# jonathanking/protein-transformer

Measured on AMD Instinct MI355X. Metric: train-step residues/sec (enc-only d512, drmsd loss), higher is better.
Workload: dtype f32 (GEMM and attention operands scaled by powers of two and split into 2 f16 terms [activation x weight products, weight-gradient products whose operands come with a uniform scale, attention with head size 64 / 32] or exactly into 3 bf16 terms [the other weight-gradient products; everything when to; 1 GPU; enc-only d_model=512 n_layers=6 n_head=8 d_ff=2048, -l drmsd, sgd lr 1e-4 wd 0.01 clip 1, dropout 0.1, 32 proteins x L=512 per GPU (BASELINE.json configs[3]); global_batch=32, seq_len=512, parallelism=dp1

## Files before the change

include/ptamd.h:

```cpp
#ifndef PTAMD_H
#define PTAMD_H

#include <stddef.h>
#include <stdint.h>

#ifdef __cplusplus
extern "C" {
#endif

#define PTAMD_OK 0
#define PTAMD_ERR_BAD_SHAPE (-1)
#define PTAMD_ERR_TOO_LONG (-2)
#define PTAMD_ERR_WORKSPACE (-3)
#define PTAMD_ERR_HIP (-4)
#define PTAMD_ERR_ALIGN (-5)

#define PTAMD_ST_BAD_RESIDUE 1
#define PTAMD_ST_TOO_SHORT 2
#define PTAMD_ST_BAD_THETA 4
#define PTAMD_ST_NONFINITE 8

#define PTAMD_PAD_ID 20
#define PTAMD_NUM_ANGLES 12
#define PTAMD_NUM_SLOTS 14
// ... 24 lines not shown

int ptamd_kabsch_rmsd(const float *pred_crd, const float *true_crd, const int64_t *seq, int B, int L, float *rmsd,
                      void *stream);

size_t ptamd_mse_angles_workspace_bytes(void);
int ptamd_mse_angles_fwd(const float *pred, const float *truth, int64_t T, float *out, void *workspace,
                         size_t workspace_bytes, void *stream);
int ptamd_mse_angles_bwd(const float *pred, const float *truth, int64_t T, const float *sums, float coef,
                         int accumulate, float *dpred, void *stream);

#define PTAMD_EPI_RELU 1
#define PTAMD_EPI_TANH 2
#define PTAMD_EPI_ACCUM 4
#define PTAMD_EPI_SLABS 16
#define PTAMD_EPI_GATE 8
typedef struct {
  int M, N, K;
  const float *A; int lda; int a_kmajor;
  const float *B; int ldb; int b_kmajor;
  float *C; int ldc;
  const float *bias;
  const float *residual; int ldr;
  int flags;
  float dropout_p; uint64_t seed; uint32_t stream_id;
  int split_k;
  void *workspace; size_t workspace_bytes;
  float *colsum;
  float gate_scale;
  int arith;
  int reserved_cus;
  const uint32_t *a_scale; int a_scale_stride;
  const uint32_t *b_scale; int b_scale_stride;
  const uint64_t *gate_mask;
} ptamd_gemm_args;
size_t ptamd_gate_mask_bytes(int M, int N);
size_t ptamd_gemm_workspace_bytes(int M, int N, int split_k);
int ptamd_gemm(const ptamd_gemm_args *args, void *stream);

#define PTAMD_GEMM_F32 0
#define PTAMD_GEMM_BF16X3 1
#define PTAMD_GEMM_BF16X3_FULL 2
#define PTAMD_GEMM_F16X2 3
#define PTAMD_GEMM_AUTO 4
int ptamd_gemm_products(const ptamd_gemm_args *args);
int ptamd_gemm_group(const ptamd_gemm_args *args, int n, void *stream);

size_t ptamd_hp_bytes(int rows, int K);
int ptamd_hp_padded_rows(int rows);
int ptamd_hp_split(const float *x, int ld, int rows, int K, int transposed, void *planes, float *scale, void *stream);
typedef struct {
  const float *x; int ld, rows, K;
  void *planes; float *scale;
} ptamd_hp_split_job;
int ptamd_hp_split_rows(const ptamd_hp_split_job *jobs_host, int njobs, void *stream);
int ptamd_hp_split_cols(const ptamd_hp_split_job *jobs_host, int njobs, void *stream);
typedef struct {
  int M, N, K;
  const void *A; const float *A_scale;
  const void *B; const float *B_scale;
  float *C; int ldc;
  const float *bias;
  const float *residual; int ldr;
  int flags;
  float dropout_p; uint64_t seed; uint32_t stream_id;
  int split_k;
  void *workspace; size_t workspace_bytes;
  float gate_scale;
  int reserved_cus;
  const uint64_t *gate_mask;
  uint64_t *gate_mask_out;
  void *kv_planes; float *kv_inv; int kv_col0, kv_heads;
} ptamd_gemm_hp_args;
size_t ptamd_gemm_hp_workspace_bytes(int M, int N, int split_k);
int ptamd_gemm_hp(const ptamd_gemm_hp_args *args, void *stream);

typedef struct {
  const float *w; int rows, cols, ld;
  uint32_t *row_scale; uint32_t *col_scale; float *stats;
  int rows_only;
} ptamd_wscale_job;
int ptamd_weight_scales(const ptamd_wscale_job *jobs_host, int njobs, void *stream);
typedef struct {
  const float *ln_gamma_stats; const float *ln_beta_stats;
  const float *w_stats; int w_stat_index;
  const float *bias_stats;
  float sqrt_d, post_scale;
  uint32_t *out_scale; float *out_value;
} ptamd_bound_job;
int ptamd_bound_scales(const ptamd_bound_job *jobs_host, int njobs, void *stream);
typedef struct { uint32_t *dst; int64_t n; uint32_t value; } ptamd_fill_job;
int ptamd_fill_u32(const ptamd_fill_job *jobs_host, int njobs, void *stream);

typedef struct {
  int64_t offset;
  int32_t rows, cols;
  int32_t stats_row0;
  int32_t stats_index;
  int32_t row_scale_index;
  int32_t col_scale_index;
  int32_t colmax_index;
  int32_t colsq_index;
  uint64_t row_planes;
  uint64_t col_planes;
  int32_t ld;
  int32_t rowmax_index;
} ptamd_wprep_seg;
typedef struct {
  int32_t ln_gamma_stats, ln_beta_stats, w_stats, w_stat_index, bias_stats;
  float sqrt_d, post_scale;
  int32_t out_scale, out_value;
} ptamd_wprep_bound;
typedef struct {
// ... 93 lines not shown
```

protein_transformer_amd/_lib.py:

```python
import ctypes as C
import os

import torch

_HERE = os.path.dirname(os.path.abspath(__file__))
_TAG = os.environ.get("PTAMD_LIB_TAG", "")
LIB_PATH = os.path.join(_HERE, "csrc", f"libptamd_{_TAG}.so" if _TAG else "libptamd.so")

OK = 0
ERRORS = {-1: "bad shape", -2: "sequence too long for the NeRF LDS staging", -3: "workspace missing or too small",
          -4: "HIP runtime error", -5: "pointer not 16-byte aligned"}
ST_BAD_RESIDUE, ST_TOO_SHORT, ST_BAD_THETA, ST_NONFINITE = 1, 2, 4, 8

_p, _i, _i64, _f, _sz, _u64, _u32 = C.c_void_p, C.c_int, C.c_int64, C.c_float, C.c_size_t, C.c_uint64, C.c_uint32


class GemmArgs(C.Structure):
    _fields_ = [("M", _i), ("N", _i), ("K", _i),
                ("A", _p), ("lda", _i), ("a_kmajor", _i),
                ("B", _p), ("ldb", _i), ("b_kmajor", _i),
                ("C", _p), ("ldc", _i),
                ("bias", _p),
                ("residual", _p), ("ldr", _i),
                ("flags", _i),
                ("dropout_p", _f), ("seed", _u64), ("stream_id", _u32),
                ("split_k", _i),
                ("workspace", _p), ("workspace_bytes", _sz),
                ("colsum", _p),
                ("gate_scale", _f),
                ("arith", _i),
                ("reserved_cus", _i),
                ("a_scale", _p), ("a_scale_stride", _i),
                ("b_scale", _p), ("b_scale_stride", _i),
                ("gate_mask", _p)]


class WScaleJob(C.Structure):
    _fields_ = [("w", _p), ("rows", _i), ("cols", _i), ("ld", _i), ("row_scale", _p), ("col_scale", _p), ("stats", _p),
                ("rows_only", _i)]


class BoundJob(C.Structure):
    _fields_ = [("ln_gamma_stats", _p), ("ln_beta_stats", _p), ("w_stats", _p), ("w_stat_index", _i), ("bias_stats", _p),
                ("sqrt_d", _f), ("post_scale", _f), ("out_scale", _p), ("out_value", _p)]


class LnReduceJob(C.Structure):
    _fields_ = [("partials", _p), ("D", _i), ("dgamma", _p), ("dbeta", _p)]


class FillJob(C.Structure):
    _fields_ = [("dst", _p), ("n", _i64), ("value", _u32)]


class HpSplitJob(C.Structure):
    _fields_ = [("x", _p), ("ld", _i), ("rows", _i), ("K", _i), ("planes", _p), ("scale", _p)]


class GemmHpArgs(C.Structure):
    _fields_ = [("M", _i), ("N", _i), ("K", _i),
                ("A", _p), ("A_scale", _p),
                ("B", _p), ("B_scale", _p),
                ("C", _p), ("ldc", _i),
                ("bias", _p),
                ("residual", _p), ("ldr", _i),
                ("flags", _i),
                ("dropout_p", _f), ("seed", _u64), ("stream_id", _u32),
                ("split_k", _i),
                ("workspace", _p), ("workspace_bytes", _sz),
                ("gate_scale", _f),
                ("reserved_cus", _i),
                ("gate_mask", _p), ("gate_mask_out", _p),
                ("kv_planes", _p), ("kv_inv", _p), ("kv_col0", _i), ("kv_heads", _i)]


class WprepSeg(C.Structure):
    _fields_ = [("offset", _i64), ("rows", C.c_int32), ("cols", C.c_int32), ("stats_row0", C.c_int32), ("stats_index", C.c_int32),
                ("row_scale_index", C.c_int32), ("col_scale_index", C.c_int32), ("colmax_index", C.c_int32),
                ("colsq_index", C.c_int32), ("row_planes", _u64), ("col_planes", _u64), ("ld", C.c_int32), ("rowmax_index", C.c_int32)]


class WprepBound(C.Structure):
    _fields_ = [("ln_gamma_stats", C.c_int32), ("ln_beta_stats", C.c_int32), ("w_stats", C.c_int32), ("w_stat_index", C.c_int32),
                ("bias_stats", C.c_int32), ("sqrt_d", _f), ("post_scale", _f), ("out_scale", C.c_int32), ("out_value", C.c_int32)]


class WprepPlan(C.Structure):
    _fields_ = [("segs", _p), ("nsegs", C.c_int32),
                ("blocks_a", _p), ("nblocks_a", C.c_int32), ("nblocks_a_matrices", C.c_int32),
                ("plain", _p), ("nplain", C.c_int32),
                ("blocks_b", _p), ("nblocks_b", C.c_int32),
                ("bounds", _p), ("nbounds", C.c_int32),
                ("groups", _p), ("ngroups", C.c_int32),
                ("colnorm_segs", _p),
                ("scales", _p), ("values", _p),
                ("colmax", _p), ("ncolmax", C.c_int32),
                ("colsq", _p),
                ("stats", _p), ("nstats", C.c_int32),
                ("numel", _i64), ("with_planes", C.c_int32)]


SIGNATURES = {
    "ptamd_version": (C.c_char_p, []),
    "ptamd_last_hip_error": (C.c_char_p, []),
    "ptamd_sidechain_atoms": (_i, [_i]),
    "ptamd_angles_fwd": (_i, [_p, _p, _i64, _p]),
# ... 133 lines not shown
```

protein_transformer_amd/csrc/gemm.hip:

```cpp
#include <stdlib.h>

#include "gemm_common.h"

namespace ptgemm {
namespace {

template <bool KMAJOR, int BK>
__device__ __forceinline__ void store_stage(float *__restrict__ s, int tid, const float4 (&v)[BK / 8]) {
  constexpr int LPR = BK / 4, LD_R = BK + 4;
#pragma unroll
  for (int i = 0; i < BK / 8; ++i) {
    if (!KMAJOR) {
      const int row = tid / LPR + (NT / LPR) * i, k = 4 * (tid % LPR);
      *reinterpret_cast<float4 *>(s + row * LD_R + k) = v[i];
    } else {
      const int k = (tid >> 5) + 8 * i, row = 4 * (tid & 31);
      *reinterpret_cast<float4 *>(s + k * LD_C + row) = v[i];
    }
  }
}
template <bool KMAJOR, int BK>
__device__ __forceinline__ void read_frag(const float *__restrict__ s, int r, int lh, int m, float (&f)[4]) {
  constexpr int LD_R = BK + 4;
  if (!KMAJOR) {
// ... 313 lines not shown
int round4(int n) { return (n + 3) & ~3; }
}

size_t ptamd_gemm_workspace_bytes(int M, int N, int split_k) {
  if (M <= 0 || N <= 0) return 0;
  return slab_bytes(M, N, split_k) + (size_t)(round4(M) + round4(N)) * sizeof(uint32_t);
}

namespace {
bool valid_arith(int mode) {
  return mode == PTAMD_GEMM_F32 || mode == PTAMD_GEMM_BF16X3 || mode == PTAMD_GEMM_BF16X3_FULL || mode == PTAMD_GEMM_F16X2 ||
         mode == PTAMD_GEMM_AUTO;
}
int resolve_mode(const ptamd_gemm_args *a) {
  int mode = a->arith;
  if (mode == PTAMD_GEMM_AUTO) mode = a->a_kmajor ? PTAMD_GEMM_BF16X3 : PTAMD_GEMM_F16X2;
  const size_t a_bytes = (size_t)(a->a_kmajor ? a->K : a->M) * a->lda * sizeof(float);
  const size_t b_bytes = (size_t)(a->b_kmajor ? a->K : a->N) * a->ldb * sizeof(float);
  if (mode == PTAMD_GEMM_F16X2 && a->K < 32) mode = PTAMD_GEMM_BF16X3;
  if (a->K < 16 || a_bytes >= ((size_t)1 << 32) || b_bytes >= ((size_t)1 << 32)) mode = PTAMD_GEMM_F32;
  return mode;
}
}

int ptamd_gemm_products(const ptamd_gemm_args *a) {
  if (!a || a->M <= 0 || a->N <= 0 || a->K <= 0 || !valid_arith(a->arith)) return PTAMD_ERR_BAD_SHAPE;
  const int mode = resolve_mode(a);
  return mode == PTAMD_GEMM_F32 ? 1 : mode == PTAMD_GEMM_F16X2 ? 3 : mode == PTAMD_GEMM_BF16X3_FULL ? 9 : 6;
}

namespace {
int build_params(const ptamd_gemm_args *a, GemmParams &p, int &splits, int &mode, float *&user_c) {
  if (!a || a->M <= 0 || a->N <= 0 || a->K <= 0 || !valid_arith(a->arith)) return PTAMD_ERR_BAD_SHAPE;
  if ((a->lda & 3) || (a->ldb & 3)) return PTAMD_ERR_BAD_SHAPE;
  if ((!a->a_kmajor || !a->b_kmajor) && (a->K & 3)) return PTAMD_ERR_BAD_SHAPE;
  if (a->a_kmajor && (a->M & 3)) return PTAMD_ERR_BAD_SHAPE;
  if (a->b_kmajor && (a->N & 3)) return PTAMD_ERR_BAD_SHAPE;
  if (!pt_aligned16(a->A) || !pt_aligned16(a->B)) return PTAMD_ERR_ALIGN;
  if (a->dropout_p < 0.f || a->dropout_p >= 1.f) return PTAMD_ERR_BAD_SHAPE;
  splits = a->split_k > 1 ? a->split_k : 1;
  constexpr int BK = 32;
  const int kblocks = (a->K + BK - 1) / BK;
  if (splits > kblocks) splits = kblocks;
  p.M = a->M; p.N = a->N; p.K = a->K;
  p.A = a->A; p.lda = a->lda; p.B = a->B; p.ldb = a->ldb; p.C = a->C; p.ldc = a->ldc;
  p.bias = a->bias; p.residual = a->residual; p.ldr = a->ldr; p.flags = a->flags & ~PTAMD_EPI_SLABS;
  if ((a->flags & PTAMD_EPI_SLABS) && (a->bias || a->residual || a->colsum || a->gate_mask || a->dropout_p != 0.f ||
                                      (a->flags & (PTAMD_EPI_RELU | PTAMD_EPI_TANH | PTAMD_EPI_ACCUM | PTAMD_EPI_GATE))))
    return PTAMD_ERR_BAD_SHAPE;
  p.dropout_p = a->dropout_p; p.seed = a->seed; p.stream_id = a->stream_id; p.gate_scale = a->gate_scale;
  p.reserved_cus = a->reserved_cus;
  p.k_per_split = ((kblocks + splits - 1) / splits) * BK;
  splits = (a->K + p.k_per_split - 1) / p.k_per_split;
  p.splits = splits;
  p.vec_epilogue = !(a->N & 3) && !(a->ldc & 3) && pt_aligned16(a->C) &&
                   (!a->residual || (!(a->ldr & 3) && pt_aligned16(a->residual))) &&
                   (splits == 1 || pt_aligned16(a->workspace));
  p.slab = 0;
  p.colsum = a->colsum;
  p.colsum_share = 1;
  {
    const int tiles_n = (a->N + BN - 1) / BN;
    while (p.colsum_share * 2 <= tiles_n && p.colsum_share < 16) p.colsum_share *= 2;
  }
  if (a->colsum && !a->a_kmajor) return PTAMD_ERR_BAD_SHAPE;
  if ((a->flags & PTAMD_EPI_GATE) && (a->residual == nullptr) == (a->gate_mask == nullptr)) return PTAMD_ERR_BAD_SHAPE;
  if (a->gate_mask && !(a->flags & PTAMD_EPI_GATE)) return PTAMD_ERR_BAD_SHAPE;
  p.gate_mask = a->gate_mask; p.gate_mask_out = nullptr;
  p.mask_rb = (a->M + 31) / 32; p.mask_cb = (a->N + 31) / 32;
  user_c = a->C;
  if (splits > 1) {
    if (!a->workspace || a->workspace_bytes < slab_bytes(a->M, a->N, splits)) return PTAMD_ERR_WORKSPACE;
    p.slab = (size_t)a->M * a->N;
    p.C = static_cast<float *>(a->workspace);
    if (a->colsum) p.colsum = p.C + (size_t)splits * p.slab;
  }
  mode = resolve_mode(a);
  if (a->gate_mask && (mode != PTAMD_GEMM_F16X2 || !p.vec_epilogue || splits > 1 || a->dropout_p != 0.f)) return PTAMD_ERR_BAD_SHAPE;
  p.scale_a = p.scale_b = nullptr;
  p.scale_a_stride = p.scale_b_stride = 1;
  if (mode == PTAMD_GEMM_F16X2) {
    if (a->a_scale && a->a_scale_stride != 0 && a->a_scale_stride != 1) return PTAMD_ERR_BAD_SHAPE;
    if (a->b_scale && a->b_scale_stride != 0 && a->b_scale_stride != 1) return PTAMD_ERR_BAD_SHAPE;
  }
  return PTAMD_OK;
}
}

size_t ptamd_gate_mask_bytes(int M, int N) {
  if (M <= 0 || N <= 0) return 0;
  return (size_t)((M + 31) / 32) * ((N + 31) / 32) * 16 * sizeof(uint64_t);
}

int ptamd_gemm(const ptamd_gemm_args *a, void *stream) {
  GemmParams p;
  int splits, mode;
  float *user_c;
  if (const int rc = build_params(a, p, splits, mode, user_c)) return rc;
  hipStream_t st = (hipStream_t)stream;
  if (mode == PTAMD_GEMM_F16X2) {
    uint32_t *sa = nullptr, *sb = nullptr;
    if (!a->a_scale || !a->b_scale) {
      if (!a->workspace || !pt_aligned16(a->workspace) || a->workspace_bytes < ptamd_gemm_workspace_bytes(a->M, a->N, splits))
        return PTAMD_ERR_WORKSPACE;
      uint32_t *ws = reinterpret_cast<uint32_t *>(static_cast<char *>(a->workspace) + slab_bytes(a->M, a->N, splits));
      if (!a->a_scale) sa = ws;
      if (!a->b_scale) sb = ws + round4(a->M);
      if (const int rs = launch_row_scales(p, a->a_kmajor != 0, a->b_kmajor != 0, sa, sb, st)) return rs;
    }
    p.scale_a = a->a_scale ? a->a_scale : sa;
// ... 60 lines not shown
```

protein_transformer_amd/csrc/gemm_common.h:

```cpp
#pragma once
#include "common.h"

namespace ptgemm {

typedef float f32x16 __attribute__((ext_vector_type(16)));
typedef float f32x4 __attribute__((ext_vector_type(4)));

constexpr int BM = 128, BN = 128, NT = 256;
constexpr int LD_C = 132;

struct GemmParams {
  int M, N, K;
  const float *A;
  int lda;
  const float *B;
  int ldb;
  float *C;
  int ldc;
  const float *bias;
  const float *residual;
  int ldr;
  int flags;
  float dropout_p;
  uint64_t seed;
  uint32_t stream_id;
  int k_per_split;
  int splits;
  size_t slab;
  int vec_epilogue;
  float *colsum;
  int colsum_share;
  float gate_scale;
  const uint32_t *scale_a, *scale_b;
  int scale_a_stride, scale_b_stride;
  int reserved_cus;
  const uint64_t *gate_mask;
  uint64_t *gate_mask_out;
  int mask_rb, mask_cb;
};
__device__ __forceinline__ uint32_t load_gate_masks(const GemmParams &p, int rb, int cb, int lane) {
  const int rbu = __builtin_amdgcn_readfirstlane(rb), cbu = __builtin_amdgcn_readfirstlane(cb);
  const bool in = rbu < p.mask_rb && cbu < p.mask_cb;
  const uint32_t *src = reinterpret_cast<const uint32_t *>(p.gate_mask + ((size_t)(in ? cbu : 0) * p.mask_rb + (in ? rbu : 0)) * 16);
  return src[lane & 31];
}
__device__ __forceinline__ bool gate_keep(uint32_t masks, int r) {
  const uint32_t lo = (uint32_t)__builtin_amdgcn_readlane((int)masks, 2 * r), hi = (uint32_t)__builtin_amdgcn_readlane((int)masks, 2 * r + 1);
  return __builtin_amdgcn_inverse_ballot_w64(((uint64_t)hi << 32) | lo);
}

template <bool KMAJOR, int BK>
__device__ __forceinline__ void load_stage(const float *__restrict__ src, int ld, int rows, int r0, int kend, int k0,
                                           int tid, float4 (&v)[BK / 8]) {
  constexpr int LPR = BK / 4;
#pragma unroll
  for (int i = 0; i < BK / 8; ++i) {
    if (!KMAJOR) {
      const int row = r0 + tid / LPR + (NT / LPR) * i, k = k0 + 4 * (tid % LPR);
      v[i] = (row < rows && k < kend) ? *reinterpret_cast<const float4 *>(src + (size_t)row * ld + k)
                                      : make_float4(0.f, 0.f, 0.f, 0.f);
    } else {
      const int k = k0 + (tid >> 5) + 8 * i, row = r0 + 4 * (tid & 31);
      v[i] = (k < kend && row < rows) ? *reinterpret_cast<const float4 *>(src + (size_t)k * ld + row)
                                      : make_float4(0.f, 0.f, 0.f, 0.f);
    }
  }
}
__device__ __forceinline__ float epilogue_value(float v, int row, int col, const GemmParams &p, uint32_t thr,
                                                float keep_scale) {
  if (p.bias) v += p.bias[col];
  if (p.flags & PTAMD_EPI_RELU) v = fmaxf(v, 0.f);
// ... 192 lines not shown
```

protein_transformer_amd/csrc/gemm_f16x2.hip:

```cpp
#include "gemm_split_kernel.h"

namespace ptgemm {
namespace {

struct ScaleJob {
  const float *x;
  int ld, rows, K, kmajor;
  uint32_t *scale;
  int blocks;
};
constexpr int RS_THREADS = 256, RS_ROWS = 8, RS_KCHUNK = 128;
constexpr int RS_KMAJOR_CHUNKS = 1, RS_KMAJOR_WHOLE = 2;

__device__ __forceinline__ float absmax4(float m, const float4 v) {
  return fmaxf(fmaxf(m, fmaxf(fabsf(v.x), fabsf(v.y))), fmaxf(fabsf(v.z), fabsf(v.w)));
}

__global__ __launch_bounds__(RS_THREADS) void gemm_row_scale_kernel(const ScaleJob ja, const ScaleJob jb) {
  const bool second = (int)blockIdx.x >= ja.blocks;
  const ScaleJob j = second ? jb : ja;
  const int b = (int)blockIdx.x - (second ? ja.blocks : 0);
  const int tid = threadIdx.x, lane = tid & 63, wave = tid >> 6;
  if (!j.kmajor) {
    for (int rr = 0; rr < RS_ROWS / 4; rr += 2) {
// ... 65 lines not shown
        m.x = fmaxf(m.x, o.x); m.y = fmaxf(m.y, o.y); m.z = fmaxf(m.z, o.z); m.w = fmaxf(m.w, o.w);
      }
      atomicMin(j.scale + r4 + 0, row_scale_bits(__float_as_uint(m.x)));
      atomicMin(j.scale + r4 + 1, row_scale_bits(__float_as_uint(m.y)));
      atomicMin(j.scale + r4 + 2, row_scale_bits(__float_as_uint(m.z)));
      atomicMin(j.scale + r4 + 3, row_scale_bits(__float_as_uint(m.w)));
    }
  }
}

}

int launch_row_scales(const GemmParams &p, bool a_kmajor, bool b_kmajor, uint32_t *scale_a, uint32_t *scale_b, hipStream_t st) {
  auto job = [](const float *x, int ld, int rows, int K, bool kmajor, uint32_t *scale) {
    const int mode = !kmajor ? 0 : ((size_t)rows * K <= ((size_t)1 << 21) ? RS_KMAJOR_WHOLE : RS_KMAJOR_CHUNKS);
    ScaleJob j = {x, ld, rows, K, mode, scale, 0};
    j.blocks = mode == RS_KMAJOR_CHUNKS  ? ((rows + 255) / 256) * ((K + RS_KCHUNK - 1) / RS_KCHUNK)
               : mode == RS_KMAJOR_WHOLE ? (rows + 15) / 16
                                         : (rows + RS_ROWS - 1) / RS_ROWS;
    return j;
  };
  ScaleJob ja = job(p.A, p.lda, p.M, p.K, a_kmajor, scale_a), jb = job(p.B, p.ldb, p.N, p.K, b_kmajor, scale_b);
  if (!scale_a) ja.blocks = 0;
  if (!scale_b) jb.blocks = 0;
  if (ja.blocks + jb.blocks == 0) return PTAMD_OK;
  if (ja.blocks && ja.kmajor == RS_KMAJOR_CHUNKS)
    PT_HIP_TRY(hipMemsetD32Async(reinterpret_cast<hipDeviceptr_t>(scale_a), (int)(254u << 23), (size_t)p.M, st));
  if (jb.blocks && jb.kmajor == RS_KMAJOR_CHUNKS)
    PT_HIP_TRY(hipMemsetD32Async(reinterpret_cast<hipDeviceptr_t>(scale_b), (int)(254u << 23), (size_t)p.N, st));
  hipLaunchKernelGGL(gemm_row_scale_kernel, dim3(ja.blocks + jb.blocks), dim3(RS_THREADS), 0, st, ja, jb);
  return pt_check_launch();
}

int launch_group_f16x2(const GemmGroup &g, hipStream_t st) { return launch_group<3>(g, st); }

int launch_split_f16x2(const GemmParams &p, bool a_kmajor, bool b_kmajor, int splits, hipStream_t st) {
  const bool plain = p.slab != 0 || (!p.bias && !p.residual && !p.flags && p.dropout_p == 0.f);
  if (plain) return launch_layout<3, EPI_PLAIN>(p, a_kmajor, b_kmajor, splits, st);
  if (p.dropout_p == 0.f) return launch_layout<3, EPI_NODROP>(p, a_kmajor, b_kmajor, splits, st);
  return launch_layout<3, EPI_FULL>(p, a_kmajor, b_kmajor, splits, st);
}

}
```

protein_transformer_amd/csrc/gemm_hp.hip:

```cpp
#include <stdlib.h>

#include "gemm_common.h"
#include "hp_format.h"
#include "kv_format.h"
#include "split_bf16.h"

extern "C" __device__ int pt_llvm_amdgcn_writelane(int value, int lane, int old) __asm("llvm.amdgcn.writelane");

namespace pthp {
namespace {

using ptgemm::GemmParams;
using ptgemm::f32x16;
using ptsplit::f16x8;

constexpr int HBN = 128;

struct HpParams {
  GemmParams g;
  const char *a_planes, *b_planes;
  const float *a_scale, *b_scale;
  int kb16;
  int a_rb_last, b_rb_last;
  char *kv_planes;
  float *kv_inv;
  int kv_col0, kv_heads, kv_nt;
};

typedef __attribute__((address_space(1))) const void *gptr_t;
typedef __attribute__((address_space(3))) void *lptr_t;
__device__ __forceinline__ void dma16(const char *g, char *l) {
  __builtin_amdgcn_global_load_lds((gptr_t)g, (lptr_t)l, 16, 0, 0);
}

struct Item {
  int bm0, bn0, z, kbeg, kend;
};
struct Cursor {
  int w, k0;
  Item it;
};

template <int WM_, int TI_, int KB_, bool ILV_>
struct HpGeom {
  static constexpr int WM = WM_, TI = TI_, KB = KB_;
  static constexpr bool ILV = ILV_;
  static constexpr int NW = 2 * WM, THREADS = 64 * NW, TILE_M = 32 * TI * WM, BK = 16 * KB;
  static constexpr int A_BLOCKS = TILE_M / 32, B_BLOCKS = HBN / 32;
  static constexpr int RB_BYTES = KB * 2048;
  static constexpr int A_STAGE = A_BLOCKS * RB_BYTES, STAGE_BYTES = (A_BLOCKS + B_BLOCKS) * RB_BYTES;
  static constexpr int PIECES = STAGE_BYTES / 1024, PER_WAVE = PIECES / NW;
  static constexpr int SCRATCH_BYTES = NW * 2048 * 4;
  static constexpr size_t LDS = (size_t)2 * STAGE_BYTES + SCRATCH_BYTES;
  static constexpr int WG_PER_CU = LDS <= 80 * 1024 ? 2 : 1;
  static_assert(PIECES % NW == 0, "pieces must divide evenly over the wavefronts");
  static_assert(LDS <= 160 * 1024, "LDS budget of a CU");
};

template <typename G, int EPI>
// ... 93 lines not shown
      }
#pragma unroll
      for (int i = 0; i < TI; ++i)
#pragma unroll
        for (int j = 0; j < 2; ++j) acc[i][j] = __builtin_amdgcn_mfma_f32_32x32x16_f16(fa[i][1], fb[j][0], acc[i][j], 0, 0, 0);
      dma_slot(PER_SLOT);
#pragma unroll
      for (int i = 0; i < TI; ++i)
#pragma unroll
        for (int j = 0; j < 2; ++j) acc[i][j] = __builtin_amdgcn_mfma_f32_32x32x16_f16(fa[i][0], fb[j][1], acc[i][j], 0, 0, 0);
      dma_slot(PER_SLOT);
#pragma unroll
      for (int i = 0; i < TI; ++i)
#pragma unroll
        for (int j = 0; j < 2; ++j) acc[i][j] = __builtin_amdgcn_mfma_f32_32x32x16_f16(fa[i][0], fb[j][0], acc[i][j], 0, 0, 0);
      dma_slot(PER_SLOT);
    }
    if (more_loads) more_loads = advance(ld);
    if (cc.k0 + BK >= cc.it.kend) {
      float *C = p.g.C + (partial ? (size_t)cc.it.z * p.g.slab : 0);
      const int ldc = partial ? p.g.N : p.g.ldc;
      const int row0 = cc.it.bm0 + wm * 32 * TI, col0 = cc.it.bn0 + wn * 64;
      {
        const int l31 = lane & 31, lh = lane >> 5;
        float ib[2];
#pragma unroll
        for (int j = 0; j < 2; ++j) ib[j] = inverse_of_scale(p.b_scale[min(col0 + j * 32 + l31, p.g.N - 1)]);
#pragma unroll
        for (int i = 0; i < TI; ++i)
#pragma unroll
          for (int g = 0; g < 4; ++g)
#pragma unroll
            for (int e = 0; e < 4; ++e) {
              const float ia = inverse_of_scale(p.a_scale[min(row0 + i * 32 + 8 * g + 4 * lh + e, p.g.M - 1)]);
#pragma unroll
              for (int j = 0; j < 2; ++j) acc[i][j][g * 4 + e] = acc[i][j][g * 4 + e] * ia * ib[j];
            }
      }
      if (p.g.vec_epilogue)
        ptgemm::tile_epilogue_vec<TI, true, EPI>(p.g, acc, C, ldc, partial, row0, col0, lane, thr, keep_scale, scratch + wave * 2048);
      else
        ptgemm::tile_epilogue_vec<TI, false, EPI>(p.g, acc, C, ldc, partial, row0, col0, lane, thr, keep_scale, scratch + wave * 2048);
      zero_acc();
    }
    if (!advance(cc)) break;
    buf ^= 1;
  }
}

template <typename G, int EPI>
int launch_hp_g(const HpParams &p, int splits, hipStream_t st) {
  const int work = ((p.g.M + G::TILE_M - 1) / G::TILE_M) * ((p.g.N + HBN - 1) / HBN) * splits;
  auto kern = gemm_hp_kernel<G, EPI>;
  PT_HIP_TRY(hipFuncSetAttribute(reinterpret_cast<const void *>(kern), hipFuncAttributeMaxDynamicSharedMemorySize, (int)G::LDS));
  const int slots = ptgemm::persistent_grid(p.g.reserved_cus) * G::WG_PER_CU;
  hipLaunchKernelGGL(kern, dim3(work < slots ? work : slots), dim3(G::THREADS), G::LDS, st, p);
  return pt_check_launch();
}

typedef HpGeom<4, 2, 2, true> Geom;

template <int EPI, bool KVP = false>
int launch_hp3(const HpParams &p, int splits, hipStream_t st);
template <int EPI>
int launch_hp(const HpParams &p, int splits, hipStream_t st) {
  if (p.g.vec_epilogue) return launch_hp3<EPI == ptgemm::EPI_NODROP ? ptgemm::EPI_FULL : EPI>(p, splits, st);
  if (p.g.gate_mask_out) return PTAMD_ERR_BAD_SHAPE;
  return launch_hp_g<Geom, EPI>(p, splits, st);
}

struct Hp3 {
  static constexpr int WM = 4, NW = 2 * WM, THREADS = 64 * NW, TILE_M = 64 * WM, BK = 32, NSTAGE = 3;
  static constexpr int A_BLOCKS = 2 * WM, B_BLOCKS = 4, PER_WAVE = (A_BLOCKS + B_BLOCKS) * 4 / NW;
  static constexpr int RB_BYTES = 4096, A_STAGE = A_BLOCKS * RB_BYTES, STAGE_BYTES = (A_BLOCKS + B_BLOCKS) * RB_BYTES;
  static constexpr int SCRATCH_BYTES = NW * 2048;
  static constexpr size_t LDS = (size_t)NSTAGE * STAGE_BYTES + SCRATCH_BYTES;
  static_assert(LDS <= 160 * 1024, "the LDS of a CU");
};

__device__ __forceinline__ void kv_split8(const float4 &a, const float4 &b, float s, uint4 &hi, uint4 &lo) {
  uint2 h0, l0, h1, l1;
  ptsplit::split_quad_f16(a.x, a.y, a.z, a.w, s, s, s, s, h0, l0);
  ptsplit::split_quad_f16(b.x, b.y, b.z, b.w, s, s, s, s, h1, l1);
  hi = make_uint4(h0.x, h0.y, h1.x, h1.y);
  lo = make_uint4(l0.x, l0.y, l1.x, l1.y);
}
__device__ __forceinline__ uint32_t half_umax(uint32_t v) {
  v = max(v, (uint32_t)__builtin_amdgcn_update_dpp(0, (int)v, 0xB1, 0xF, 0xF, true));
  v = max(v, (uint32_t)__builtin_amdgcn_update_dpp(0, (int)v, 0x4E, 0xF, 0xF, true));
  v = max(v, (uint32_t)__builtin_amdgcn_update_dpp(0, (int)v, 0x141, 0xF, 0xF, true));
  v = max(v, (uint32_t)__builtin_amdgcn_update_dpp(0, (int)v, 0x140, 0xF, 0xF, true));
  v = max(v, (uint32_t)__shfl_xor((int)v, 16, 64));
  return v;
}

template <int EPI, bool KVP = false>
__device__ __forceinline__ void hp3_epilogue(const GemmParams &p, const f32x16 (&acc)[2][2], float *C, int ldc, bool partial,
                                             int row0, int col0, int lane, uint32_t thr, float keep_scale, float *scratch,
                                             const HpParams *hp = nullptr) {
  using ptgemm::EPI_FULL;
  using ptgemm::EPI_PLAIN;
  typedef float f32x4 __attribute__((ext_vector_type(4)));
  const int l31 = lane & 31, lh = lane >> 5;
  uint32_t keep[2] = {0xffffffffu, 0xffffffffu};
  if (EPI == EPI_FULL && !partial && p.dropout_p > 0.f) {
    keep[0] = keep[1] = 0u;
#pragma unroll 4
    for (int idx = 0; idx < 8; ++idx) {
      const int i = idx >> 2, j = (idx >> 1) & 1, gp = idx & 1;
      const int row = row0 + i * 32 + 16 * gp + 4 * lh, col = col0 + j * 32 + l31;
      const uint4 rnd = pt_rand4(p.seed, drop_call_index(row, col, p.N), p.stream_id);
      const uint32_t t16 = thr >> 16;
      uint32_t bits = 0;
#pragma unroll
      for (int f = 0; f < 8; ++f)
        bits |= (drop_field_value(rnd, f) >= t16 ? 1u : 0u) << (j * 16 + (2 * gp + (f >> 2)) * 4 + (f & 3));
      keep[0] |= i == 0 ? bits : 0u;
      keep[1] |= i == 1 ? bits : 0u;
    }
  }
#pragma unroll
  for (int i = 0; i < 2; ++i) {
    __builtin_amdgcn_sched_barrier(0);
    f32x4 pre4[8];
    const bool want_res = EPI != EPI_PLAIN && !partial && p.residual != nullptr;
    const bool want_old = EPI != EPI_PLAIN && !partial && (p.flags & PTAMD_EPI_ACCUM) && !want_res;
#pragma unroll
    for (int t = 0; t < 8; ++t) {
      const int f = lane + 64 * t, rr = f >> 4, c4 = (f & 15) * 4;
      const int row = min(row0 + i * 32 + rr, p.M - 1), col = min(col0 + c4, p.N - 4);
      const float *src = want_res ? p.residual + (size_t)row * p.ldr + col : C + (size_t)row * ldc + col;
      pre4[t] = (f32x4){0.f, 0.f, 0.f, 0.f};
      if (want_res || want_old) pre4[t] = *reinterpret_cast<const f32x4 *>(src);
    }
    float bias[2];
#pragma unroll
// ... 21 lines not shown
            if (EPI == EPI_FULL && p.dropout_p > 0.f) v = (keep[i] >> (j * 16 + g * 4 + e)) & 1u ? v * keep_scale : 0.f;
            if (gated) v = ptgemm::gate_keep(gmk[j], g * 4 + e) ? v * p.gate_scale : 0.f;
            if (p.gate_mask_out) {
              const uint64_t m = __builtin_amdgcn_ballot_w64(v > 0.f);
              mask_lo[j] = pt_llvm_amdgcn_writelane((int)(uint32_t)m, g * 4 + e, mask_lo[j]);
              mask_hi[j] = pt_llvm_amdgcn_writelane((int)(uint32_t)(m >> 32), g * 4 + e, mask_hi[j]);
            }
          }
          scratch[(4 * lh + e) * 64 + j * 32 + l31] = v;
        }
      if (KVP && col0 >= hp->kv_col0) {
        const int rr = lane >> 3, ch = lane & 7;
        const float4 a = *reinterpret_cast<const float4 *>(scratch + rr * 64 + ch * 8);
        const float4 b = *reinterpret_cast<const float4 *>(scratch + rr * 64 + ch * 8 + 4);
        const uint32_t am = half_umax(max(max(max(__float_as_uint(a.x) & 0x7fffffffu, __float_as_uint(a.y) & 0x7fffffffu),
                                              max(__float_as_uint(a.z) & 0x7fffffffu, __float_as_uint(a.w) & 0x7fffffffu)),
                                          max(max(__float_as_uint(b.x) & 0x7fffffffu, __float_as_uint(b.y) & 0x7fffffffu),
                                              max(__float_as_uint(b.z) & 0x7fffffffu, __float_as_uint(b.w) & 0x7fffffffu))));
        const uint32_t sbits = pt_row_scale_bits(am);
        uint4 hi, lo;
        kv_split8(a, b, __uint_as_float(sbits), hi, lo);
        const int hc = (col0 - hp->kv_col0) >> 6;
        const int gt = (row0 >> 5) + i, r = 8 * g + rr;
        if (row0 + i * 32 < p.M) {
          char *tile = hp->kv_planes + ((size_t)hc * hp->kv_nt + gt) * ptkv::TILE_BYTES;
          char *dst = tile + r * ptkv::ROW_BYTES + ptkv::chunk_pos(r, ch) * 16;
          *reinterpret_cast<uint4 *>(dst) = hi;
          *reinterpret_cast<uint4 *>(dst + ptkv::PLANE_BYTES) = lo;
          if ((lane & 31) == 0)
            hp->kv_inv[((size_t)hc * hp->kv_nt + gt) * 8 + ptkv::group_slot(2 * g + lh)] = __uint_as_float((254u << 23) - sbits);
        }
        continue;
      }
#pragma unroll
      for (int u = 0; u < 2; ++u) {
        const int f = lane + 64 * u, rr = f >> 4, c4 = (f & 15) * 4;
        const int row = row0 + i * 32 + 8 * g + rr, col = col0 + c4;
        float4 v = *reinterpret_cast<const float4 *>(scratch + rr * 64 + c4);
#ifdef PT_ABLATE_NOSTORE
        if (row < p.M && col < p.N && p.M < 0) {
#else
        if (row < p.M && col < p.N) {
#endif
          if (EPI != EPI_PLAIN && !partial) {
            const f32x4 r4 = pre4[2 * g + u];
            if (p.residual) {
              if (p.flags & PTAMD_EPI_GATE) {
                v.x = r4.x > 0.f ? v.x * p.gate_scale : 0.f; v.y = r4.y > 0.f ? v.y * p.gate_scale : 0.f;
                v.z = r4.z > 0.f ? v.z * p.gate_scale : 0.f; v.w = r4.w > 0.f ? v.w * p.gate_scale : 0.f;
              } else {
                v.x += r4.x; v.y += r4.y; v.z += r4.z; v.w += r4.w;
              }
            }
            if (p.flags & PTAMD_EPI_TANH) { v.x = tanhf(v.x); v.y = tanhf(v.y); v.z = tanhf(v.z); v.w = tanhf(v.w); }
            if (p.flags & PTAMD_EPI_ACCUM) {
              const f32x4 o4 = want_old ? r4 : *reinterpret_cast<const f32x4 *>(C + (size_t)row * ldc + col);
              v.x += o4.x; v.y += o4.y; v.z += o4.z; v.w += o4.w;
            }
          }
          *reinterpret_cast<float4 *>(C + (size_t)row * ldc + col) = v;
        }
      }
    }
    if (EPI != EPI_PLAIN && !partial && p.gate_mask_out) {
      const int rb = __builtin_amdgcn_readfirstlane((row0 >> 5) + i);
#pragma unroll
      for (int j = 0; j < 2; ++j) {
        const int cb = __builtin_amdgcn_readfirstlane((col0 >> 5) + j);
        if (lane < 16 && rb < p.mask_rb && cb < p.mask_cb)
          p.gate_mask_out[((size_t)cb * p.mask_rb + rb) * 16 + lane] = ((uint64_t)(uint32_t)mask_hi[j] << 32) | (uint32_t)mask_lo[j];
      }
    }
  }
}

#define PT_DS_READ_B128(dst, addr, off) asm volatile("ds_read_b128 %0, %1 offset:%2" : "=v"(dst) : "v"(addr), "n"(off))

template <int EPI, bool KVP = false>
__global__ __launch_bounds__(Hp3::THREADS, 2) void gemm_hp3_kernel(const HpParams p) {
  using G = Hp3;
  extern __shared__ __attribute__((aligned(16))) char smem[];
  float *const scratch = reinterpret_cast<float *>(smem + G::NSTAGE * G::STAGE_BYTES);
  const int tid = threadIdx.x, lane = tid & 63;
  const int wave = __builtin_amdgcn_readfirstlane(tid >> 6);
  const int wm = wave >> 1, wn = wave & 1;
  const ptgemm::WorkRange work(p.g, G::TILE_M, HBN);
  if (work.begin >= work.end) return;
  const int Kp = p.kb16 * 16;
  auto item_at = [&](int logical) __attribute__((always_inline)) {
    Item it;
    work.decode(logical, it.bm0, it.bn0, it.z);
    it.kbeg = it.z * p.g.k_per_split;
    it.kend = min(Kp, it.kbeg + p.g.k_per_split);
    return it;
  };
  auto advance = [&](Cursor &c) __attribute__((always_inline)) {
    if (c.k0 + G::BK < c.it.kend) {
      c.k0 += G::BK;
      return true;
    }
    if (c.w + 1 < work.end) {
      c.it = item_at(++c.w);
      c.k0 = c.it.kbeg;
      return true;
    }
    return false;
  };
  const int rb_in_tile = wave >> 2, rest_bytes = (wave & 3) * 1024;
  const char *const a_base = p.a_planes + rest_bytes + lane * 16, *const b_base = p.b_planes + rest_bytes + lane * 16;
  const int64_t row_bytes = (int64_t)p.kb16 * 2048;
  auto issue_piece = [&](const Cursor &c, int buf, int i) __attribute__((always_inline)) {
// ... 73 lines not shown
        const int ta = pr == 0 ? 1 : 0, tb = pr == 1 ? 1 : 0;
#pragma unroll
        for (int i = 0; i < 2; ++i)
#pragma unroll
          for (int j = 0; j < 2; ++j)
            acc[i][j] = __builtin_amdgcn_mfma_f32_32x32x16_f16(fa[kb][i][ta], fb[kb][j][tb], acc[i][j], 0, 0, 0);
        __builtin_amdgcn_sched_barrier(0);
        if (issue) issue_piece(ld, nbuf, kb * 3 + pr);
        __builtin_amdgcn_sched_barrier(0);
      }
    }
    if (issue) {
      more_loads = advance(ld);
      ++ahead;
    }
    --ahead;
    if (cc.k0 + G::BK >= cc.it.kend) {
      asm volatile("s_waitcnt vmcnt(0)" ::: "memory");
      landed = ahead;
      float *C = p.g.C + (partial ? (size_t)cc.it.z * p.g.slab : 0);
      const int ldc = partial ? p.g.N : p.g.ldc;
      const int row0 = cc.it.bm0 + wm * 64, col0 = cc.it.bn0 + wn * 64;
      {
        const int l31 = lane & 31, lh = lane >> 5;
        float ib[2];
#pragma unroll
        for (int j = 0; j < 2; ++j) ib[j] = inverse_of_scale(p.b_scale[min(col0 + j * 32 + l31, p.g.N - 1)]);
#pragma unroll
        for (int i = 0; i < 2; ++i)
#pragma unroll
          for (int g = 0; g < 4; ++g)
#pragma unroll
            for (int e = 0; e < 4; ++e) {
              const float ia = inverse_of_scale(p.a_scale[min(row0 + i * 32 + 8 * g + 4 * lh + e, p.g.M - 1)]);
#pragma unroll
              for (int j = 0; j < 2; ++j) acc[i][j][g * 4 + e] = acc[i][j][g * 4 + e] * ia * ib[j];
            }
      }
      hp3_epilogue<EPI, KVP>(p.g, acc, C, ldc, partial, row0, col0, lane, thr, keep_scale, scratch + wave * 512, &p);
      zero_acc();
    }
    if (!advance(cc)) break;
    buf = buf == G::NSTAGE - 1 ? 0 : buf + 1;
  }
}

template <int EPI, bool KVP>
int launch_hp3(const HpParams &p, int splits, hipStream_t st) {
  const int work = ((p.g.M + Hp3::TILE_M - 1) / Hp3::TILE_M) * ((p.g.N + HBN - 1) / HBN) * splits;
  auto kern = gemm_hp3_kernel<EPI, KVP>;
  PT_HIP_TRY(hipFuncSetAttribute(reinterpret_cast<const void *>(kern), hipFuncAttributeMaxDynamicSharedMemorySize, (int)Hp3::LDS));
  const int slots = ptgemm::persistent_grid(p.g.reserved_cus);
  hipLaunchKernelGGL(kern, dim3(work < slots ? work : slots), dim3(Hp3::THREADS), Hp3::LDS, st, p);
  return pt_check_launch();
}

__global__ __launch_bounds__(256) void hp_rowscale_kernel(const float *__restrict__ x, int ld, int rows, int K, int rows_p,
                                                          float *__restrict__ scale) {
  const int r = blockIdx.x * 4 + (threadIdx.x >> 6), lane = threadIdx.x & 63;
  if (r >= rows_p) return;
  if (r >= rows) {
    if (lane == 0) scale[r] = 1.f;
    return;
  }
  const float *p = x + (size_t)r * ld;
  float m = 0.f;
  for (int k = lane * 4; k < K; k += 256) {
    const float4 v = *reinterpret_cast<const float4 *>(p + k);
    m = fmaxf(fmaxf(m, fmaxf(fabsf(v.x), fabsf(v.y))), fmaxf(fabsf(v.z), fabsf(v.w)));
  }
  m = wave_max(m);
  if (lane == 0) scale[r] = __uint_as_float(scale_bits_of(__float_as_uint(m)));
}
__global__ __launch_bounds__(256) void hp_colmax_kernel(const float *__restrict__ x, int ld, int rows, int K,
                                                        uint32_t *__restrict__ amax) {
  const int r = blockIdx.x * 256 + threadIdx.x;
  if (r >= rows) return;
  const int k0 = blockIdx.y * 64, k1 = min(K, k0 + 64);
  float m = 0.f;
  for (int k = k0; k < k1; ++k) m = fmaxf(m, fabsf(x[(size_t)k * ld + r]));
  atomicMax(amax + r, __float_as_uint(m));
}
__global__ __launch_bounds__(256) void hp_amax_to_scale_kernel(uint32_t *__restrict__ amax_scale, int rows, int rows_p) {
// ... 181 lines not shown
  j.njobs = njobs;
  hipStream_t st = (hipStream_t)stream;
  if (kmax <= 256) hipLaunchKernelGGL(hp_split_rows_kernel<1>, dim3(blocks), dim3(256), 0, st, j);
  else if (kmax <= 512) hipLaunchKernelGGL(hp_split_rows_kernel<2>, dim3(blocks), dim3(256), 0, st, j);
  else if (kmax <= 1024) hipLaunchKernelGGL(hp_split_rows_kernel<4>, dim3(blocks), dim3(256), 0, st, j);
  else hipLaunchKernelGGL(hp_split_rows_kernel<8>, dim3(blocks), dim3(256), 0, st, j);
  return pt_check_launch();
}

int ptamd_hp_split_cols(const ptamd_hp_split_job *jobs, int njobs, void *stream) {
  if (!jobs || njobs <= 0 || njobs > MAX_SPLIT_JOBS) return PTAMD_ERR_BAD_SHAPE;
  SplitColsJobs j;
  int blocks = 0;
  for (int i = 0; i < njobs; ++i) {
    const ptamd_hp_split_job &q = jobs[i];
    if (!q.x || !q.planes || !q.scale || q.rows <= 0 || q.K <= 0 || q.ld < q.rows) return PTAMD_ERR_BAD_SHAPE;
    if (!pt_aligned16(q.planes)) return PTAMD_ERR_ALIGN;
    j.x[i] = q.x; j.planes[i] = static_cast<char *>(q.planes); j.scale[i] = q.scale;
    j.ld[i] = q.ld; j.rows[i] = q.rows; j.K[i] = q.K;
    j.first_block[i] = blocks;
    const int64_t nchunks = (int64_t)(round_up(q.rows, 32) / 32) * kb16(q.K) * 64;
    blocks += (int)((nchunks + 255) / 256);
  }
  for (int i = njobs; i <= MAX_SPLIT_JOBS; ++i) j.first_block[i] = blocks;
  j.njobs = njobs;
  hipLaunchKernelGGL(hp_split_cols_kernel, dim3(blocks), dim3(256), 0, (hipStream_t)stream, j);
  return pt_check_launch();
}

size_t ptamd_gemm_hp_workspace_bytes(int M, int N, int split_k) { return (M <= 0 || N <= 0) ? 0 : slab_bytes(M, N, split_k); }

int ptamd_gemm_hp(const ptamd_gemm_hp_args *a, void *stream) {
  if (!a || a->M <= 0 || a->N <= 0 || a->K <= 0) return PTAMD_ERR_BAD_SHAPE;
  if (!a->A || !a->B || !a->A_scale || !a->B_scale || !a->C) return PTAMD_ERR_BAD_SHAPE;
  if (!pt_aligned16(a->A) || !pt_aligned16(a->B)) return PTAMD_ERR_ALIGN;
  if (a->dropout_p < 0.f || a->dropout_p >= 1.f) return PTAMD_ERR_BAD_SHAPE;
  if ((a->flags & PTAMD_EPI_GATE) && (a->residual == nullptr) == (a->gate_mask == nullptr)) return PTAMD_ERR_BAD_SHAPE;
  if (a->gate_mask && !(a->flags & PTAMD_EPI_GATE)) return PTAMD_ERR_BAD_SHAPE;
  HpParams p;
  GemmParams &g = p.g;
  g.M = a->M; g.N = a->N; g.K = a->K;
  g.A = nullptr; g.lda = 0; g.B = nullptr; g.ldb = 0; g.C = a->C; g.ldc = a->ldc;
  g.bias = a->bias; g.residual = a->residual; g.ldr = a->ldr; g.flags = a->flags;
  g.dropout_p = a->dropout_p; g.seed = a->seed; g.stream_id = a->stream_id; g.gate_scale = a->gate_scale;
  g.reserved_cus = a->reserved_cus;
  g.colsum = nullptr; g.colsum_share = 1; g.scale_a = g.scale_b = nullptr; g.scale_a_stride = g.scale_b_stride = 1;
  g.gate_mask = a->gate_mask; g.gate_mask_out = a->gate_mask_out;
  g.mask_rb = (a->M + 31) / 32; g.mask_cb = (a->N + 31) / 32;
  constexpr int HBK = 32;
  const int Kp = round_up(a->K, 32), stages = Kp / HBK;
  int splits = a->split_k > 1 ? a->split_k : 1;
  if (splits > stages) splits = stages;
  g.k_per_split = ((stages + splits - 1) / splits) * HBK;
  splits = (Kp + g.k_per_split - 1) / g.k_per_split;
  g.splits = splits;
  g.vec_epilogue = !(a->N & 3) && !(a->ldc & 3) && pt_aligned16(a->C) &&
                   (!a->residual || (!(a->ldr & 3) && pt_aligned16(a->residual))) && (splits == 1 || pt_aligned16(a->workspace));
  g.slab = 0;
  float *user_c = a->C;
  if (splits > 1) {
    if (!a->workspace || a->workspace_bytes < slab_bytes(a->M, a->N, splits)) return PTAMD_ERR_WORKSPACE;
    g.slab = (size_t)a->M * a->N;
    g.C = static_cast<float *>(a->workspace);
  }
  p.a_planes = static_cast<const char *>(a->A);
  p.b_planes = static_cast<const char *>(a->B);
  p.a_scale = a->A_scale;
  p.b_scale = a->B_scale;
  p.kb16 = Kp / 16;
  p.a_rb_last = (round_up(a->M, 32) / 32) - 1;
  p.b_rb_last = (round_up(a->N, 32) / 32) - 1;
  p.kv_planes = static_cast<char *>(a->kv_planes);
  p.kv_inv = a->kv_inv;
  p.kv_col0 = a->kv_col0;
  p.kv_heads = a->kv_heads;
  p.kv_nt = a->M / 32;
  hipStream_t st = (hipStream_t)stream;
  if (a->kv_planes) {
    if (!a->kv_inv || a->kv_heads <= 0 || (a->M & 31) || (a->kv_col0 & 63) || a->kv_col0 < 0 ||
        a->N != a->kv_col0 + 2 * a->kv_heads * 64 || !g.vec_epilogue || splits > 1 || a->residual || a->gate_mask ||
        a->gate_mask_out || a->dropout_p != 0.f || a->flags != 0)
      return PTAMD_ERR_BAD_SHAPE;
    if (!pt_aligned16(a->kv_planes)) return PTAMD_ERR_ALIGN;
    return launch_hp3<ptgemm::EPI_FULL, true>(p, 1, st);
  }
  const bool plain = !a->bias && !a->residual && !a->gate_mask && !a->gate_mask_out &&
                     !(a->flags & (PTAMD_EPI_RELU | PTAMD_EPI_TANH | PTAMD_EPI_ACCUM)) && a->dropout_p == 0.f;
  if ((a->gate_mask || a->gate_mask_out) && (!g.vec_epilogue || splits > 1)) return PTAMD_ERR_BAD_SHAPE;
  int rc;
  if (plain || splits > 1) rc = launch_hp<ptgemm::EPI_PLAIN>(p, splits, st);
  else if (a->dropout_p == 0.f) rc = launch_hp<ptgemm::EPI_NODROP>(p, splits, st);
  else rc = launch_hp<ptgemm::EPI_FULL>(p, splits, st);
  if (rc || splits == 1) return rc;
  const float *slabs = g.C;
  g.C = user_c;
  return ptgemm::launch_splitk_reduce(g, slabs, splits, nullptr, nullptr, st);
}

}
```

protein_transformer_amd/csrc/gemm_split_kernel.h:

```cpp
#pragma once
#include <type_traits>

#include <stdlib.h>

#include "gemm_common.h"
#include "split_bf16.h"

namespace ptgemm {
namespace {

using namespace ptsplit;

constexpr int TBN = 128;
constexpr int NTHREADS = 512, NPRODUCER = 256;
constexpr int KR_PAD = 32;
constexpr int SCRATCH_FLOATS = 4 * 2048;
constexpr int COLSUM_AREAS = 3;
constexpr int COLSUM_FLOATS = COLSUM_AREAS * 4 * 256;
constexpr int cmax(int a, int b) { return a > b ? a : b; }

template <int NPROD, int TI = 4>
struct Geo {
  static constexpr int TBM = 64 * TI;
  static constexpr bool F16 = NPROD == 3;
// ... 77 lines not shown
    if (!KMAJOR) soff[i] = (uint32_t)min(r0 + pt / G::QK + (NPRODUCER / G::QK) * (i < NV ? i : 0), rows - 1) * 4u * (uint32_t)stride;
    else soff[i] = (uint32_t)min(r0 + 4 * (pt % LPK), rows - 4) * 4u * (uint32_t)stride;
  }
}
template <typename G, bool KMAJOR, int ROWS>
__device__ __forceinline__ void load_scales(const uint32_t *__restrict__ scale, const uint32_t (&soff)[MAX_NV], float (&sc)[MAX_NV]) {
  const char *base = reinterpret_cast<const char *>(scale);
  constexpr int NV = G::template nv<ROWS>();
  if (!KMAJOR) {
#pragma unroll
    for (int i = 0; i < NV; ++i) sc[i] = *reinterpret_cast<const float *>(base + soff[i]);
  } else {
    const float4 v = *reinterpret_cast<const float4 *>(base + soff[0]);
    sc[0] = v.x; sc[1] = v.y; sc[2] = v.z; sc[3] = v.w;
  }
}
template <typename G, bool KMAJOR, int ROWS>
__device__ __forceinline__ void store_split_f16_one(unsigned short *__restrict__ s, int pt, const float4 &v, const float (&sc)[MAX_NV], int i) {
  constexpr int LPK = ROWS / 4, PLANE = G::template plane<ROWS>(), LD_KR = ROWS + KR_PAD;
  const int kl = KMAJOR ? pt / LPK + (NPRODUCER / LPK) * i : 4 * (pt % G::QK);
  uint2 t1, t2;
  split_quad_f16(v.x, v.y, v.z, v.w, KMAJOR ? sc[0] : sc[i], KMAJOR ? sc[1] : sc[i], KMAJOR ? sc[2] : sc[i], KMAJOR ? sc[3] : sc[i], t1, t2);
  const int off = KMAJOR ? kl * LD_KR + 4 * (pt % LPK) : G::rk_offset(pt / G::QK + (NPRODUCER / G::QK) * i, kl);
  *reinterpret_cast<uint2 *>(s + off) = t1;
  *reinterpret_cast<uint2 *>(s + PLANE + off) = t2;
}
template <typename G, bool KMAJOR, int ROWS>
__device__ __forceinline__ void store_split_f16(unsigned short *__restrict__ s, int pt, const float4 (&v)[G::template nv<ROWS>()],
                                                const float (&sc)[MAX_NV]) {
  constexpr int NV = G::template nv<ROWS>();
#pragma unroll
  for (int i = 0; i < NV; ++i) store_split_f16_one<G, KMAJOR, ROWS>(s, pt, v[i], sc, i);
}
__device__ __forceinline__ uint32_t row_scale_bits(uint32_t amax) { return min(268u - (amax >> 23), 254u) << 23; }
__device__ __forceinline__ float inverse_scale(uint32_t scale_bits) { return __uint_as_float((254u << 23) - scale_bits); }

template <typename G, bool KMAJOR, int ROWS>
__device__ __forceinline__ bf16x8 read_frag(const unsigned short *__restrict__ s, int r0, int lane, int t, int ks) {
  constexpr int PLANE = G::template plane<ROWS>(), LD_KR = ROWS + KR_PAD;
  if (!KMAJOR) {
    return *reinterpret_cast<const bf16x8 *>(s + t * PLANE + G::rk_offset(r0 + (lane & 31), 16 * ks + 8 * (lane >> 5)));
  } else {
    const int q16 = lane & 15;
    const unsigned short *q = s + t * PLANE + (16 * ks + 8 * (lane >> 5) + (q16 >> 2)) * LD_KR + r0 + (lane & 16) + 4 * (q16 & 3);
    const s16x4 lo = __builtin_amdgcn_ds_read_tr16_b64_v4i16((lds_s16x4 *)q);
    const s16x4 hi = __builtin_amdgcn_ds_read_tr16_b64_v4i16((lds_s16x4 *)(q + 4 * LD_KR));
    const s16x8 both = __builtin_shufflevector(lo, hi, 0, 1, 2, 3, 4, 5, 6, 7);
    return __builtin_bit_cast(bf16x8, both);
  }
}

struct Item {
  int bm0, bn0, z, kbeg, kend, pj;
};

struct Cursor {
  int w, k0;
  Item it;
  bool end;
};

template <bool GROUPED>
struct KernelArg {
  typedef GemmParams type;
};
template <>
struct KernelArg<true> {
  typedef GemmGroup type;
};
template <bool A_KMAJOR, bool B_KMAJOR, int NPROD, int EPI, int TI = 4, bool GROUPED = false>
__global__ __launch_bounds__(NTHREADS, 1) __attribute__((amdgpu_waves_per_eu(2, 2))) void gemm_bf16x3_mfma_kernel(
    const typename KernelArg<GROUPED>::type arg) {
  extern __shared__ __attribute__((aligned(16))) unsigned short smem[];
  using G = Geo<NPROD, TI>;
  constexpr int TBM = G::TBM;
  static_assert(TI == 4 || !A_KMAJOR, "the fused bias gradient of k-major A assumes 256-row tiles");
  constexpr int SBK = G::SBK, NSETS = G::NSETS, STAGE = G::STAGE, PLANE_A = G::PLANE_A, NVA = G::NVA, NVB = G::NVB;
  float *const scratch = reinterpret_cast<float *>(smem + 2 * STAGE);
  float *const cs_area = scratch + SCRATCH_FLOATS;

  constexpr bool F16 = NPROD == 3;
  const int tid = threadIdx.x, lane = tid & 63, wave = tid >> 6;
  auto P = [&](int j) __attribute__((always_inline)) -> const GemmParams & {
    if constexpr (GROUPED) return arg.p[j];
    else return arg;
  };
  typename std::conditional<GROUPED, GroupRange, WorkRange>::type work(arg, TBM, TBN);
  if (work.begin >= work.end) return;
  auto item_at = [&](int logical) __attribute__((always_inline)) {
    Item it;
    if constexpr (GROUPED) work.decode(arg, logical, it.pj, it.bm0, it.bn0, it.z);
    else {
      work.decode(logical, it.bm0, it.bn0, it.z);
      it.pj = 0;
    }
    it.kbeg = it.z * P(it.pj).k_per_split;
    it.kend = min(P(it.pj).K, it.kbeg + P(it.pj).k_per_split);
    return it;
  };
  auto advance = [&](Cursor &c) __attribute__((always_inline)) {
    if (c.k0 + SBK < c.it.kend) {
      c.k0 += SBK;
    } else if (c.w + 1 < work.end) {
      c.it = item_at(++c.w);
      c.k0 = c.it.kbeg;
    } else {
      c.end = true;
    }
  };
  int total_stages = 0;
  for (int w = work.begin; w < work.end; ++w) {
    const Item it = item_at(w);
    total_stages += (it.kend - it.kbeg + SBK - 1) / SBK;
  }
  const int padded_stages = (total_stages + NSETS - 1) / NSETS * NSETS;
  const bool partial = P(0).slab != 0;
  const bool has_colsum = A_KMAJOR && P(0).colsum != nullptr;
  auto cs_share_of = [&](const Item &it) __attribute__((always_inline)) { return partial ? P(it.pj).colsum_share : 1; };
  auto colsum_first = [&](const Item &it) __attribute__((always_inline)) { return (it.bn0 / TBN) & (cs_share_of(it) - 1); };
  auto colsum_on = [&](const Item &it) __attribute__((always_inline)) {
    return has_colsum && (partial ? it.bn0 / TBN < cs_share_of(it) : it.bn0 == 0);
  };

  if (wave >= 4) {
    const int pt = tid - NPRODUCER;
    float4 csum = make_float4(0.f, 0.f, 0.f, 0.f);
    float cs_w[NVA];
#pragma unroll
    for (int i = 0; i < NVA; ++i) cs_w[i] = 0.f;
    int cs_parity = 0;
    auto colsum_weights = [&](const Item &it) __attribute__((always_inline)) {
      const bool on = colsum_on(it);
      const int first = colsum_first(it), cs_share = cs_share_of(it);
#pragma unroll
      for (int i = 0; i < NVA; ++i) cs_w[i] = (on && ((pt / 64 + 4 * i) & (cs_share - 1)) == first) ? 1.f : 0.f;
    };

    Cursor ld = {work.begin, 0, item_at(work.begin), false};
    ld.k0 = ld.it.kbeg;
    Cursor st = ld;
    colsum_weights(st.it);
    uint32_t voa[NVA], vob[NVB];
    const float *opA = P(ld.it.pj).A, *opB = P(ld.it.pj).B;
    int op_lda = P(ld.it.pj).lda, op_ldb = P(ld.it.pj).ldb;
    item_offsets<G, A_KMAJOR, TBM>(op_lda, P(ld.it.pj).M, ld.it.bm0, pt, voa);
    item_offsets<G, B_KMAJOR, TBN>(op_ldb, P(ld.it.pj).N, ld.it.bn0, pt, vob);
    float4 ra[NSETS][NVA], rb[NSETS][NVB];
    float rsa[NSETS][MAX_NV], rsb[NSETS][MAX_NV];
    uint32_t soa[MAX_NV], sob[MAX_NV];
    if (F16) {
      scale_offsets<G, A_KMAJOR, TBM>(P(ld.it.pj).M, ld.it.bm0, pt, soa, P(ld.it.pj).scale_a_stride);
      scale_offsets<G, B_KMAJOR, TBN>(P(ld.it.pj).N, ld.it.bn0, pt, sob, P(ld.it.pj).scale_b_stride);
    }
    int rskip[NSETS];
    auto fetch_tail = [&](float (&sa_)[MAX_NV], float (&sb_)[MAX_NV]) __attribute__((always_inline)) {
      if (F16 && ld.k0 - ld.it.kbeg < NSETS * SBK) {
        load_scales<G, A_KMAJOR, TBM>(P(ld.it.pj).scale_a, soa, sa_);
        load_scales<G, B_KMAJOR, TBN>(P(ld.it.pj).scale_b, sob, sb_);
      }
      const int w_before = ld.w;
      advance(ld);
      if (ld.w != w_before) {
        if (GROUPED) {
          opA = P(ld.it.pj).A; opB = P(ld.it.pj).B;
          op_lda = P(ld.it.pj).lda; op_ldb = P(ld.it.pj).ldb;
        }
        item_offsets<G, A_KMAJOR, TBM>(op_lda, P(ld.it.pj).M, ld.it.bm0, pt, voa);
        item_offsets<G, B_KMAJOR, TBN>(op_ldb, P(ld.it.pj).N, ld.it.bn0, pt, vob);
        if (F16) {
          scale_offsets<G, A_KMAJOR, TBM>(P(ld.it.pj).M, ld.it.bm0, pt, soa, P(ld.it.pj).scale_a_stride);
          scale_offsets<G, B_KMAJOR, TBN>(P(ld.it.pj).N, ld.it.bn0, pt, sob, P(ld.it.pj).scale_b_stride);
        }
      }
    };
    auto fetch = [&](float4 (&a)[NVA], float4 (&b)[NVB], int &kskip, float (&sa_)[MAX_NV], float (&sb_)[MAX_NV]) __attribute__((always_inline)) {
      const int klim = ld.it.kend - ld.k0;
      const int ks = klim >= SBK ? ld.k0 : ld.it.kend - SBK;
      kskip = ld.k0 - ks;
      load_raw(opA + (A_KMAJOR ? (size_t)ks * op_lda : (size_t)ks), voa, a);
      load_raw(opB + (B_KMAJOR ? (size_t)ks * op_ldb : (size_t)ks), vob, b);
      fetch_tail(sa_, sb_);
    };
    auto produce = [&](float4 (&a)[NVA], float4 (&b)[NVB], int &kskip, float (&sa_)[MAX_NV], float (&sb_)[MAX_NV], int buf) __attribute__((always_inline)) {
      unsigned short *sa = smem + buf * STAGE, *sb = sa + G::NPLANES * PLANE_A;
      mask_tail<G, A_KMAJOR, TBM>(pt, a, kskip);
      mask_tail<G, B_KMAJOR, TBN>(pt, b, kskip);
      if (has_colsum) {
#pragma unroll
        for (int i = 0; i < NVA; ++i) {
          csum.x = fmaf(cs_w[i], a[i].x, csum.x); asm volatile("" : "+v"(csum.x));
          csum.y = fmaf(cs_w[i], a[i].y, csum.y); asm volatile("" : "+v"(csum.y));
          csum.z = fmaf(cs_w[i], a[i].z, csum.z); asm volatile("" : "+v"(csum.z));
          csum.w = fmaf(cs_w[i], a[i].w, csum.w); asm volatile("" : "+v"(csum.w));
        }
      }
      if (F16) {
        const int klim = ld.it.kend - ld.k0;
        const int ks_next = klim >= SBK ? ld.k0 : ld.it.kend - SBK;
        const float *na = opA + (A_KMAJOR ? (size_t)ks_next * op_lda : (size_t)ks_next);
        const float *nb = opB + (B_KMAJOR ? (size_t)ks_next * op_ldb : (size_t)ks_next);
        constexpr int GRP = 2;
#pragma unroll
        for (int i0 = 0; i0 < NVA; i0 += GRP) {
#pragma unroll
          for (int i = i0; i < i0 + GRP && i < NVA; ++i) store_split_f16_one<G, A_KMAJOR, TBM>(sa, pt, a[i], sa_, i);
          __builtin_amdgcn_sched_barrier(0);
#pragma unroll
          for (int i = i0; i < i0 + GRP && i < NVA; ++i)
            a[i] = *reinterpret_cast<const float4 *>(reinterpret_cast<const char *>(na) + voa[i]);
          __builtin_amdgcn_sched_barrier(0);
        }
#pragma unroll
        for (int i0 = 0; i0 < NVB; i0 += GRP) {
#pragma unroll
          for (int i = i0; i < i0 + GRP && i < NVB; ++i) store_split_f16_one<G, B_KMAJOR, TBN>(sb, pt, b[i], sb_, i);
          __builtin_amdgcn_sched_barrier(0);
#pragma unroll
          for (int i = i0; i < i0 + GRP && i < NVB; ++i)
            b[i] = *reinterpret_cast<const float4 *>(reinterpret_cast<const char *>(nb) + vob[i]);
          __builtin_amdgcn_sched_barrier(0);
        }
        kskip = ld.k0 - ks_next;
      } else {
        store_split<G, A_KMAJOR, TBM>(sa, pt, a);
        store_split<G, B_KMAJOR, TBN>(sb, pt, b);
      }
      if (has_colsum && !st.end && st.k0 + SBK >= st.it.kend) {
        if (colsum_on(st.it)) {
          reinterpret_cast<float4 *>(cs_area + cs_parity * 4 * TBM)[pt] = csum;
          cs_parity = cs_parity == COLSUM_AREAS - 1 ? 0 : cs_parity + 1;
        }
        csum = make_float4(0.f, 0.f, 0.f, 0.f);
      }
      {
        const int w_before = st.w;
        const bool was_end = st.end;
        advance(st);
        if (st.w != w_before) colsum_weights(st.it);
        if (st.end && !was_end) {
#pragma unroll
          for (int i = 0; i < NVA; ++i) cs_w[i] = 0.f;
        }
      }
      __builtin_amdgcn_sched_barrier(0);
      if (F16) fetch_tail(sa_, sb_);
      else fetch(a, b, kskip, sa_, sb_);
    };
#pragma unroll
    for (int u = 0; u < NSETS; ++u) {
      fetch(ra[u], rb[u], rskip[u], rsa[u], rsb[u]);
      __builtin_amdgcn_sched_barrier(0);
    }
    produce(ra[0], rb[0], rskip[0], rsa[0], rsb[0], 0);
    __syncthreads();
    for (int g = 0; g < padded_stages; g += NSETS) {
#pragma unroll
      for (int u = 1; u <= NSETS; ++u) {
        produce(ra[u % NSETS], rb[u % NSETS], rskip[u % NSETS], rsa[u % NSETS], rsb[u % NSETS], u & 1);
        __syncthreads();
      }
    }
  } else {
    const int wm = wave >> 1, wn = wave & 1;
    f32x16 acc[TI][2];
    auto zero_acc = [&]() __attribute__((always_inline)) {
#pragma unroll
      for (int i = 0; i < TI; ++i)
#pragma unroll
        for (int j = 0; j < 2; ++j)
#pragma unroll
          for (int r = 0; r < 16; ++r) acc[i][j][r] = 0.f;
// ... 65 lines not shown
          for (int j = 0; j < 2; ++j) ib[j] = inverse_scale(p.scale_b[min(col0 + j * 32 + l31, p.N - 1) * p.scale_b_stride]);
#pragma unroll
          for (int i = 0; i < TI; ++i)
#pragma unroll
            for (int g = 0; g < 4; ++g)
#pragma unroll
              for (int e = 0; e < 4; ++e) {
                const float ia = inverse_scale(p.scale_a[min(row0 + i * 32 + 8 * g + 4 * lh + e, p.M - 1) * p.scale_a_stride]);
#pragma unroll
                for (int j = 0; j < 2; ++j) acc[i][j][g * 4 + e] = acc[i][j][g * 4 + e] * ia * ib[j];
              }
        }
        if (p.vec_epilogue) tile_epilogue_vec<TI, true, EPI, NPROD == 3 && EPI == EPI_NODROP>(p, acc, C, ldc, partial, row0, col0, lane, thr, keep_scale, scratch + wave * 2048);
        else tile_epilogue_vec<TI, false, EPI>(p, acc, C, ldc, partial, row0, col0, lane, thr, keep_scale, scratch + wave * 2048);
        zero_acc();
        if (colsum_on(cc.it)) {
          const float *q = cs_area + cs_parity * 4 * TBM;
          const int row = cc.it.bm0 + tid;
          if (row < p.M) {
            const float tot = q[tid] + q[TBM + tid] + q[2 * TBM + tid] + q[3 * TBM + tid];
            if (partial) p.colsum[((size_t)cc.it.z * cs_share + colsum_first(cc.it)) * p.M + row] = tot;
            else p.colsum[row] += tot;
          }
          cs_parity = cs_parity == COLSUM_AREAS - 1 ? 0 : cs_parity + 1;
        }
      }
      advance(cc);
    }
  }
}

constexpr int TI1_COST_X10 = 4;
constexpr int TI2_COST_NUM = 3, TI2_COST_DEN = 5;
template <bool AK, bool BKM, int NPROD, int EPI, int TI>
int launch_ti(const GemmParams &p, int splits, hipStream_t st) {
  using G = Geo<NPROD, TI>;
  const int work = ((p.M + G::TBM - 1) / G::TBM) * ((p.N + TBN - 1) / TBN) * splits;
  auto kern = gemm_bf16x3_mfma_kernel<AK, BKM, NPROD, EPI, TI>;
  PT_HIP_TRY(hipFuncSetAttribute(reinterpret_cast<const void *>(kern), hipFuncAttributeMaxDynamicSharedMemorySize,
                                 (int)G::LDS_BYTES));
  const int slots = persistent_grid(p.reserved_cus);
  const int grid = work < slots ? work : slots;
  hipLaunchKernelGGL(kern, dim3(grid), dim3(NTHREADS), G::LDS_BYTES, st, p);
  return pt_check_launch();
}
template <bool AK, bool BKM, int NPROD, int EPI>
int launch(const GemmParams &p, int splits, hipStream_t st) {
  if (!AK && NPROD != 9 && p.M > 128) {
    const int slots = persistent_grid(p.reserved_cus), nt = (p.N + TBN - 1) / TBN * splits;
    const int rounds4 = (((p.M + 255) / 256) * nt + slots - 1) / slots, rounds2 = (((p.M + 127) / 128) * nt + slots - 1) / slots;
    if constexpr (NPROD == 3) {
      const int rounds1 = (((p.M + 63) / 64) * nt + slots - 1) / slots;
      if (TI1_COST_X10 * rounds1 < 2 * TI2_COST_NUM * rounds2 && TI1_COST_X10 * rounds1 < 2 * TI2_COST_DEN * rounds4)
        return launch_ti<false, BKM, NPROD, EPI, 1>(p, splits, st);
    }
#if defined(PT_FORCE_TI)
    if (PT_FORCE_TI == 2) return launch_ti<false, BKM, NPROD, EPI, 2>(p, splits, st);
#else
    if (TI2_COST_NUM * rounds2 < TI2_COST_DEN * rounds4) return launch_ti<false, BKM, NPROD, EPI, 2>(p, splits, st);
#endif
  }
  return launch_ti<AK, BKM, NPROD, EPI, 4>(p, splits, st);
}

template <int NPROD>
int launch_group(const GemmGroup &g, hipStream_t st) {
  using G = Geo<NPROD, 4>;
  auto kern = gemm_bf16x3_mfma_kernel<true, true, NPROD, EPI_PLAIN, 4, true>;
  PT_HIP_TRY(hipFuncSetAttribute(reinterpret_cast<const void *>(kern), hipFuncAttributeMaxDynamicSharedMemorySize,
                                 (int)G::LDS_BYTES));
  const int slots = persistent_grid(g.p[0].reserved_cus), work = g.first[g.n];
  hipLaunchKernelGGL(kern, dim3(work < slots ? work : slots), dim3(NTHREADS), G::LDS_BYTES, st, g);
  return pt_check_launch();
}

template <int NPROD, int EPI>
int launch_layout(const GemmParams &p, bool ak, bool bk, int splits, hipStream_t st) {
  if (!ak && !bk) return launch<false, false, NPROD, EPI>(p, splits, st);
  if (!ak && bk) return launch<false, true, NPROD, EPI>(p, splits, st);
  if (ak && !bk) return launch<true, false, NPROD, EPI>(p, splits, st);
  return launch<true, true, NPROD, EPI>(p, splits, st);
}

}

}
```

protein_transformer_amd/csrc/scales.hip:

```cpp
#include "common.h"

namespace {

constexpr int MAX_JOBS = 40;
struct WJobs {
  ptamd_wscale_job job[MAX_JOBS];
  int first_block[MAX_JOBS + 1];
  int row_blocks[MAX_JOBS];
  int n;
};

__global__ void wscale_init_kernel(const WJobs js) {
  const int j = blockIdx.x * blockDim.x + threadIdx.x;
  if (j < js.n && js.job[j].stats) {
    float *s = js.job[j].stats;
    s[0] = s[1] = s[2] = s[3] = 0.f;
  }
}

constexpr int COLS_PER_BLOCK = 64, ROWS_PER_BLOCK = 32, WS_THREADS = 1024, WS_WAVES = WS_THREADS / 64, WS_RY = WS_THREADS / 16;
__global__ __launch_bounds__(WS_THREADS) void wscale_kernel(const WJobs js) {
  int j = 0;
  while (j + 1 < js.n && (int)blockIdx.x >= js.first_block[j + 1]) ++j;
  const ptamd_wscale_job jb = js.job[j];
  const int b = (int)blockIdx.x - js.first_block[j];
  const int tid = threadIdx.x, lane = tid & 63, wave = tid >> 6;
  uint32_t *stat_bits = reinterpret_cast<uint32_t *>(jb.stats);
  const bool vec = !(jb.cols & 3) && !(jb.ld & 3) && !(reinterpret_cast<uintptr_t>(jb.w) & 15);
  if (b < js.row_blocks[j]) {
    __shared__ float s_nrm[WS_WAVES], s_amx[WS_WAVES];
    float bn = 0.f, bm = 0.f;
    for (int rr = 0; rr < ROWS_PER_BLOCK / WS_WAVES; ++rr) {
      const int r = b * ROWS_PER_BLOCK + wave * (ROWS_PER_BLOCK / WS_WAVES) + rr;
      if (r >= jb.rows) break;
      const float *p = jb.w + (size_t)r * jb.ld;
      float m = 0.f, sq = 0.f;
      if (vec) {
        for (int c = lane * 4; c < jb.cols; c += 256) {
          const float4 v = *reinterpret_cast<const float4 *>(p + c);
          m = fmaxf(fmaxf(m, fmaxf(fabsf(v.x), fabsf(v.y))), fmaxf(fabsf(v.z), fabsf(v.w)));
          sq = fmaf(v.x, v.x, fmaf(v.y, v.y, fmaf(v.z, v.z, fmaf(v.w, v.w, sq))));
        }
      } else {
        for (int c = lane; c < jb.cols; c += 64) {
          const float v = p[c];
          m = fmaxf(m, fabsf(v));
          sq = fmaf(v, v, sq);
        }
      }
      m = wave_max(m);
      sq = wave_sum(sq);
      if (lane == 0 && jb.row_scale) jb.row_scale[r] = pt_row_scale_bits(__float_as_uint(m));
      bn = fmaxf(bn, sqrtf(sq));
      bm = fmaxf(bm, m);
    }
    if (stat_bits) {
      if (lane == 0) {
        s_nrm[wave] = bn;
        s_amx[wave] = bm;
      }
      __syncthreads();
      if (tid == 0) {
        float n = 0.f, a = 0.f;
#pragma unroll
        for (int k = 0; k < WS_WAVES; ++k) {
          n = fmaxf(n, s_nrm[k]);
          a = fmaxf(a, s_amx[k]);
        }
        atomicMax(stat_bits + 0, __float_as_uint(n));
        atomicMax(stat_bits + 2, __float_as_uint(a));
// ... 80 lines not shown
    *reinterpret_cast<uint4 *>(f.dst + i) = make_uint4(f.value, f.value, f.value, f.value);
  } else {
    for (int64_t k = i; k < f.n && k < i + 4; ++k) f.dst[k] = f.value;
  }
}

}

extern "C" {

int ptamd_fill_u32(const ptamd_fill_job *jobs, int njobs, void *stream) {
  if (!jobs || njobs <= 0 || njobs > MAX_FILLS) return PTAMD_ERR_BAD_SHAPE;
  FJobs js;
  js.n = njobs;
  int blocks = 0;
  for (int j = 0; j < njobs; ++j) {
    if (!jobs[j].dst || jobs[j].n <= 0) return PTAMD_ERR_BAD_SHAPE;
    js.job[j] = jobs[j];
    js.first_block[j] = blocks;
    blocks += (int)((jobs[j].n + 4 * FILL_THREADS - 1) / (4 * FILL_THREADS));
  }
  js.first_block[njobs] = blocks;
  hipLaunchKernelGGL(fill_u32_kernel, dim3(blocks), dim3(FILL_THREADS), 0, (hipStream_t)stream, js);
  return pt_check_launch();
}

int ptamd_weight_scales(const ptamd_wscale_job *jobs, int njobs, void *stream) {
  if (!jobs || njobs <= 0 || njobs > MAX_JOBS) return PTAMD_ERR_BAD_SHAPE;
  WJobs js;
  js.n = njobs;
  int blocks = 0;
  for (int j = 0; j < njobs; ++j) {
    const ptamd_wscale_job &q = jobs[j];
    if (!q.w || q.rows <= 0 || q.cols <= 0 || q.ld < q.cols) return PTAMD_ERR_BAD_SHAPE;
    js.job[j] = q;
    js.first_block[j] = blocks;
    js.row_blocks[j] = (q.row_scale || q.stats) ? (q.rows + ROWS_PER_BLOCK - 1) / ROWS_PER_BLOCK : 0;
    blocks += js.row_blocks[j] + (((q.col_scale || q.stats) && !q.rows_only) ? (q.cols + COLS_PER_BLOCK - 1) / COLS_PER_BLOCK : 0);
  }
  js.first_block[njobs] = blocks;
  hipStream_t st = (hipStream_t)stream;
  hipLaunchKernelGGL(wscale_init_kernel, dim3(1), dim3(64), 0, st, js);
  if (blocks > 0) hipLaunchKernelGGL(wscale_kernel, dim3(blocks), dim3(WS_THREADS), 0, st, js);
  return pt_check_launch();
}

int ptamd_bound_scales(const ptamd_bound_job *jobs, int njobs, void *stream) {
  if (!jobs || njobs <= 0 || njobs > MAX_JOBS) return PTAMD_ERR_BAD_SHAPE;
  BJobs js;
  js.n = njobs;
  for (int j = 0; j < njobs; ++j) {
    if (!jobs[j].w_stats || jobs[j].w_stat_index < 0 || jobs[j].w_stat_index > 2) return PTAMD_ERR_BAD_SHAPE;
    js.job[j] = jobs[j];
  }
  hipLaunchKernelGGL(bound_kernel, dim3(1), dim3(64), 0, (hipStream_t)stream, js);
  return pt_check_launch();
}

}
```

protein_transformer_amd/csrc/wprep.hip:

```cpp
#include "common.h"
#include "hp_format.h"
#include "optim_update.h"
#include "split_bf16.h"

namespace {

constexpr int RB = 32, WAVES = 4, RW = RB / WAVES, MAXV = 2;
constexpr int PLAIN_F4 = 4096;

struct OptArgs {
  int kind;
  int zero_g;
  float *g;
  float *m, *v;
  const float *sqnorm;
  float max_norm, lr, wd, beta1, beta2, eps, step_size, inv_sqrt_bc2;
};

using ptopt::clip_coef;
using ptopt::sgd_update;
__device__ __forceinline__ float adam_update(float p, float g, float &m, float &v, float coef, const OptArgs &o) {
  return ptopt::adam_update(p, g, m, v, coef, o.wd, o.beta1, o.beta2, o.eps, o.step_size, o.inv_sqrt_bc2);
}
template <int KIND>
// ... 233 lines not shown
    }
    return;
  }
  if (blk.x == 1) {
    if (!pl.with_planes) return;
    const ptamd_wprep_seg sg = pl.segs[blk.y];
    const int rows = sg.cols, K = sg.rows, kbv = pthp::kb16(K), ld = sg.ld;
    const int64_t nchunks = (int64_t)(pthp::round_up(rows, 32) / 32) * kbv * 64;
    const int64_t id = (int64_t)blk.z * 256 + tid;
    if (id >= nchunks) return;
    const int c = (int)(id & 63);
    const int64_t b = id >> 6;
    const int kb = (int)(b % kbv), rb = (int)(b / kbv);
    int r, h;
    pthp::chunk_coords(c, r, h);
    const int row = rb * 32 + r, k0 = kb * 16 + h * 8;
    float v[8];
#pragma unroll
    for (int e = 0; e < 8; ++e) v[e] = 0.f;
    float sc = 1.f;
    if (row < rows) {
      sc = __uint_as_float(pt_row_scale_bits(pl.colmax[sg.colmax_index + row]));
      const float *x = w + sg.offset;
#pragma unroll
      for (int e = 0; e < 8; ++e)
        if (k0 + e < K) v[e] = x[(size_t)(k0 + e) * ld + row];
    }
    uint4 hi, lo;
    ptsplit::split_pair_f16(v[0], v[1], sc, sc, hi.x, lo.x);
    ptsplit::split_pair_f16(v[2], v[3], sc, sc, hi.y, lo.y);
    ptsplit::split_pair_f16(v[4], v[5], sc, sc, hi.z, lo.z);
    ptsplit::split_pair_f16(v[6], v[7], sc, sc, hi.w, lo.w);
    char *dst = reinterpret_cast<char *>(sg.col_planes) + pthp::block_offset(rb, kb, 0, kbv) + c * 16;
    *reinterpret_cast<uint4 *>(dst) = hi;
    *reinterpret_cast<uint4 *>(dst + pthp::BLK_BYTES) = lo;
    return;
  }
  const int4 grp = pl.groups[blk.y];
  __shared__ float s_red[4];
  for (int e = 0; e < grp.w; ++e) {
    const ptamd_wprep_seg sg = pl.segs[pl.colnorm_segs[grp.z + e]];
    const int nb = (sg.rows + RB - 1) / RB;
    float nmax = 0.f;
    for (int c = tid; c < sg.cols; c += 256) {
      const double *q = pl.colsq + sg.colsq_index + c;
      double s0 = 0.0, s1 = 0.0, s2 = 0.0, s3 = 0.0;
      int b = 0;
      for (; b + 8 <= nb; b += 8) {
        double t[8];
#pragma unroll
        for (int u = 0; u < 8; ++u) t[u] = q[(int64_t)(b + u) * sg.cols];
        s0 += t[0]; s1 += t[1]; s2 += t[2]; s3 += t[3];
        s0 += t[4]; s1 += t[5]; s2 += t[6]; s3 += t[7];
      }
      for (; b < nb; ++b) s0 += q[(int64_t)b * sg.cols];
      nmax = fmaxf(nmax, (float)sqrt((s0 + s1) + (s2 + s3)));
    }
    nmax = wave_max(nmax);
    __syncthreads();
    if ((tid & 63) == 0) s_red[tid >> 6] = nmax;
    __syncthreads();
    if (tid == 0) pl.stats[4 * sg.stats_index + 1] = fmaxf(pl.stats[4 * sg.stats_index + 1], fmaxf(fmaxf(s_red[0], s_red[1]), fmaxf(s_red[2], s_red[3])));
  }
  __syncthreads();
  __threadfence_block();
  if (tid < grp.y) {
// ... 89 lines not shown
```

protein_transformer_amd/kernels.py:

```python
import ctypes as C
import os

import torch

from . import _lib
from ._lib import GemmArgs, GemmHpArgs, check, lib, ptr, stream, workspace

EPI_RELU, EPI_TANH, EPI_ACCUM, EPI_GATE, EPI_SLABS = 1, 2, 4, 8, 16

GEMM_TIMING = None
GEMM_EVENT_POOL = []
GEMM_BYTES = []
GEMM_RESERVED_CUS = 0


def gemm(A, B, C_out, *, M, N, K, lda, ldb, ldc, a_kmajor=False, b_kmajor=False, bias=None, residual=None,
         ldr=0, flags=0, dropout_p=0.0, seed=0, stream_id=0, split_k=1, colsum=None, gate_scale=0.0, arith=None,
         a_scale=None, a_scale_stride=1, b_scale=None, b_scale_stride=1, gate_mask=None, ws=None):
    if ws is None:
        ws = workspace("gemm", lib().ptamd_gemm_workspace_bytes(M, N, split_k), A.device)
    args = GemmArgs(M=M, N=N, K=K, A=A.data_ptr(), lda=lda, a_kmajor=int(a_kmajor), B=B.data_ptr(), ldb=ldb,
                    b_kmajor=int(b_kmajor), C=C_out.data_ptr() if C_out is not None else ws.data_ptr(), ldc=ldc,
                    bias=bias.data_ptr() if bias is not None else None,
                    residual=residual.data_ptr() if residual is not None else None, ldr=ldr, flags=flags,
                    dropout_p=float(dropout_p), seed=int(seed) & (2 ** 64 - 1), stream_id=int(stream_id),
                    split_k=int(split_k), workspace=ws.data_ptr() if ws is not None else None,
                    workspace_bytes=ws.numel() if ws is not None else 0,
                    colsum=colsum.data_ptr() if colsum is not None else None, gate_scale=float(gate_scale),
                    arith=int(_DEFAULT_ARITH if arith is None else arith), reserved_cus=int(GEMM_RESERVED_CUS),
                    a_scale=a_scale.data_ptr() if a_scale is not None else None, a_scale_stride=int(a_scale_stride),
                    b_scale=b_scale.data_ptr() if b_scale is not None else None, b_scale_stride=int(b_scale_stride),
                    gate_mask=gate_mask.data_ptr() if gate_mask is not None else None)
    if GEMM_TIMING is None:
        check(lib().ptamd_gemm(C.byref(args), stream()), "gemm")
    else:
        e0, e1 = GEMM_EVENT_POOL.pop(), GEMM_EVENT_POOL.pop()
        e0.record()
        check(lib().ptamd_gemm(C.byref(args), stream()), "gemm")
        e1.record()
        nprod = lib().ptamd_gemm_products(C.byref(args))
        kind = "dW" if (a_kmajor and b_kmajor) else ("dX" if b_kmajor else "fwd")
        GEMM_TIMING.append((2.0 * M * N * K, e0, e1, nprod,
                            f"ptamd_gemm {kind} (staging kernel, A_KMAJOR={int(bool(a_kmajor))} B_KMAJOR={int(bool(b_kmajor))} NPROD={nprod})"))
        GEMM_BYTES.append(4 * (M * K + N * K + M * N * (1 + (residual is not None) + bool(flags & EPI_ACCUM))))
    return C_out


GEMM_F32, GEMM_BF16X3, GEMM_BF16X3_FULL, GEMM_F16X2, GEMM_AUTO = 0, 1, 2, 3, 4




def _env_arith():
    import os
    try:
        v = int(os.environ.get("PTAMD_GEMM_MODE", GEMM_AUTO))
    except ValueError:
        v = GEMM_AUTO
    return v if v in (GEMM_F32, GEMM_BF16X3, GEMM_BF16X3_FULL, GEMM_F16X2, GEMM_AUTO) else GEMM_AUTO


_DEFAULT_ARITH = _env_arith()


def set_gemm_mode(mode):
    global _DEFAULT_ARITH
    if int(mode) not in (GEMM_F32, GEMM_BF16X3, GEMM_BF16X3_FULL, GEMM_F16X2, GEMM_AUTO):
        raise ValueError(f"unknown GEMM arithmetic {mode}")
    _DEFAULT_ARITH = int(mode)


def get_gemm_mode():
    return _DEFAULT_ARITH


class HpOperand:
    __slots__ = ("planes", "scale", "rows", "K")

    def __init__(self, rows, K, device):
        self.rows, self.K = int(rows), int(K)
        self.planes = torch.empty(lib().ptamd_hp_bytes(self.rows, self.K), dtype=torch.uint8, device=device)
        self.scale = torch.empty(lib().ptamd_hp_padded_rows(self.rows), dtype=torch.float32, device=device)


def hp_split(x, transposed=False, out=None):
    assert x.dim() == 2 and x.stride(1) == 1
    rows, K = (x.shape[1], x.shape[0]) if transposed else (x.shape[0], x.shape[1])
    if out is None:
        out = HpOperand(rows, K, x.device)
    check(lib().ptamd_hp_split(ptr(x), x.stride(0), rows, K, int(transposed), ptr(out.planes), ptr(out.scale), stream()),
          "hp_split")
    return out


def gemm_hp(a, b, C_out, *, bias=None, residual=None, ldr=0, flags=0, dropout_p=0.0, seed=0, stream_id=0, split_k=1,
            gate_scale=0.0, gate_mask=None, gate_mask_out=None, kv=None, kv_col0=0, kv_heads=0):
    assert a.K == b.K
    M, N = a.rows, b.rows
    ws = workspace("gemm_hp", lib().ptamd_gemm_hp_workspace_bytes(M, N, split_k), C_out.device) if split_k > 1 else None
    args = GemmHpArgs(M=M, N=N, K=a.K, A=a.planes.data_ptr(), A_scale=a.scale.data_ptr(), B=b.planes.data_ptr(),
                      B_scale=b.scale.data_ptr(), C=C_out.data_ptr(), ldc=C_out.stride(0),
                      bias=bias.data_ptr() if bias is not None else None,
                      residual=residual.data_ptr() if residual is not None else None, ldr=ldr, flags=flags,
                      dropout_p=float(dropout_p), seed=int(seed) & (2 ** 64 - 1), stream_id=int(stream_id),
                      split_k=int(split_k), workspace=ws.data_ptr() if ws is not None else None,
                      workspace_bytes=ws.numel() if ws is not None else 0, gate_scale=float(gate_scale),
                      reserved_cus=int(GEMM_RESERVED_CUS),
                      gate_mask=gate_mask.data_ptr() if gate_mask is not None else None,
                      gate_mask_out=gate_mask_out.data_ptr() if gate_mask_out is not None else None,
                      kv_planes=kv[0].data_ptr() if kv is not None else None, kv_inv=kv[1].data_ptr() if kv is not None else None,
                      kv_col0=int(kv_col0), kv_heads=int(kv_heads))
    if GEMM_TIMING is None:
        check(lib().ptamd_gemm_hp(C.byref(args), stream()), "gemm_hp")
    else:
        e0, e1 = GEMM_EVENT_POOL.pop(), GEMM_EVENT_POOL.pop()
        e0.record()
        check(lib().ptamd_gemm_hp(C.byref(args), stream()), "gemm_hp")
        e1.record()
        GEMM_TIMING.append((2.0 * M * N * a.K, e0, e1, 3, "ptamd_gemm_hp (LDS-DMA kernel gemm_hp3_kernel, NPROD=3)"))
        GEMM_BYTES.append(4 * (M * a.K + N * a.K + M * N * (1 + (residual is not None) + bool(flags & EPI_ACCUM))))
    return C_out


DW_SLOTS = 512


def pick_split_k(M, N, K, slots=None):
    slots = DW_SLOTS if slots is None else slots
    tiles = ((M + 127) // 128) * ((N + 127) // 128)
    if tiles >= slots // 2 or K <= 512:
        return 1
    return max(1, min(K // 256, slots // tiles))


SPLIT_K_ROWS = True


def pick_split_k_rows(M, N, K, slots=256):
    tiles = ((M + 127) // 128) * ((N + 127) // 128)
    if not SPLIT_K_ROWS or tiles * 2 > slots or K < 1024:
        return 1
    return max(1, min(K // 512, slots // tiles))


def linear_fwd(x, w, b, out=None, defer_reduce=False, **epi):
    T, K = x.shape
    N = w.shape[0]
    sk = pick_split_k_rows(T, N, K)
    if defer_reduce and DEFER_REDUCE and sk > 1 and out is None and b is not None and N % 4 == 0 and N <= 512 and \
            epi.get("flags", 0) == 0 and epi.get("residual") is not None and epi.get("ldr") == N and \
            epi["residual"].is_contiguous() and int(_DEFAULT_ARITH if epi.get("arith") is None else epi["arith"]) != GEMM_F32:
        n = effective_splits(K, sk)
        if 2 <= n <= 4:
            ws = workspace("gemm_slabs", lib().ptamd_gemm_workspace_bytes(T, N, sk), x.device)
# ... 59 lines not shown
                     **scales):
    T, N = dy.shape
    K = w.shape[1]
    sk = pick_split_k_rows(T, K, N)
    if defer_reduce and DEFER_REDUCE and sk > 1 and out is None and gate is None and gate_mask is None and flags == 0 and \
            K % 4 == 0 and K <= 512 and int(_DEFAULT_ARITH if arith is None else arith) != GEMM_F32:
        n = effective_splits(N, sk)
        if 2 <= n <= 4:
            ws = workspace("gemm_slabs", lib().ptamd_gemm_workspace_bytes(T, K, sk), dy.device)
            gemm(dy, w, None, M=T, N=K, K=N, lda=dy.stride(0), ldb=w.stride(0), ldc=K, b_kmajor=True, split_k=sk,
                 flags=EPI_SLABS, arith=arith, ws=ws, **scales)
            return Slabs(ws, n, T * K, (T, K))
    if out is None:
        out = torch.empty(T, K, dtype=torch.float32, device=dy.device)
    if gate_mask is not None and sk == 1 and K % 4 == 0 and out.stride(0) % 4 == 0 and out.data_ptr() % 16 == 0 and \
            int(_DEFAULT_ARITH if arith is None else arith) in (GEMM_F16X2, GEMM_AUTO) and N >= 32 and \
            dy.shape[0] * dy.stride(0) * 4 < 2 ** 32 and w.shape[0] * w.stride(0) * 4 < 2 ** 32:
        return gemm(dy, w, out, M=T, N=K, K=N, lda=dy.stride(0), ldb=w.stride(0), ldc=out.stride(0), b_kmajor=True, split_k=1,
                    flags=flags | EPI_GATE, gate_mask=gate_mask, gate_scale=1.0 / (1.0 - gate_dropout_p), arith=arith, **scales)
    if gate_mask is not None and gate is None:
        raise ValueError("linear_bwd_input: gate_mask given, but this product cannot read it (split-K, arithmetic, alignment "
                         "or operand size) and no fp32 `gate` was passed to fall back on")
    if gate is not None:
        return gemm(dy, w, out, M=T, N=K, K=N, lda=dy.stride(0), ldb=w.stride(0), ldc=out.stride(0), b_kmajor=True, split_k=sk,
                    flags=flags | EPI_GATE, residual=gate, ldr=gate.stride(0), gate_scale=1.0 / (1.0 - gate_dropout_p),
                    arith=arith, **scales)
    return gemm(dy, w, out, M=T, N=K, K=N, lda=dy.stride(0), ldb=w.stride(0), ldc=out.stride(0), b_kmajor=True, split_k=sk,
                flags=flags, arith=arith, **scales)


def linear_bwd_weight(dy, x, dw, dbias=None, arith=None, dy_scale=None, x_scale=None):
    T, N = dy.shape
    K = x.shape[1]
    if dy_scale is not None and x_scale is not None:
        return gemm(dy, x, dw, M=N, N=K, K=T, lda=dy.stride(0), ldb=x.stride(0), ldc=dw.stride(0), a_kmajor=True,
                    b_kmajor=True, flags=EPI_ACCUM, split_k=pick_split_k(N, K, T), colsum=dbias, arith=GEMM_F16X2,
                    a_scale=dy_scale, a_scale_stride=0, b_scale=x_scale, b_scale_stride=0)
    return gemm(dy, x, dw, M=N, N=K, K=T, lda=dy.stride(0), ldb=x.stride(0), ldc=dw.stride(0), a_kmajor=True,
                b_kmajor=True, flags=EPI_ACCUM, split_k=pick_split_k(N, K, T), colsum=dbias, arith=arith)


GROUP_MIN_K = int(os.environ.get("PTAMD_GROUP_MIN_K", 1024))


def pick_group_split(tiles256, T, slots=256):
    best, best_cost = 0, None
    for s in range(2, max(2, T // GROUP_MIN_K) + 1):
        rounds = -(-tiles256 * s // slots)
        cost = rounds * (-(-T // s) + 640)
        if best_cost is None or cost < best_cost:
            best, best_cost = s, cost
    return best if T >= 2048 else 0


def linear_bwd_weight_group(jobs, split_k):
    arr = (GemmArgs * len(jobs))()
    flops = 0.0
    nbytes = 0
    for j, (dy, x, dw, dbias, dy_scale, x_scale) in enumerate(jobs):
        T, N = dy.shape
        Kd = x.shape[1]
        ws = workspace(f"gemm_group{j}", lib().ptamd_gemm_workspace_bytes(N, Kd, split_k), dw.device)
        arr[j] = GemmArgs(M=N, N=Kd, K=T, A=dy.data_ptr(), lda=dy.stride(0), a_kmajor=1, B=x.data_ptr(), ldb=x.stride(0),
                          b_kmajor=1, C=dw.data_ptr(), ldc=dw.stride(0), bias=None, residual=None, ldr=0, flags=EPI_ACCUM,
                          dropout_p=0.0, seed=0, stream_id=0, split_k=int(split_k), workspace=ws.data_ptr(),
                          workspace_bytes=ws.numel(), colsum=dbias.data_ptr() if dbias is not None else None, gate_scale=0.0,
                          arith=GEMM_F16X2, reserved_cus=int(GEMM_RESERVED_CUS), a_scale=dy_scale.data_ptr(), a_scale_stride=0,
                          b_scale=x_scale.data_ptr(), b_scale_stride=0)
        flops += 2.0 * N * Kd * T
        nbytes += 4 * (N * T + Kd * T + 2 * N * Kd)
    if GEMM_TIMING is None:
        check(lib().ptamd_gemm_group(arr, len(jobs), stream()), "gemm_group")
    else:
        e0, e1 = GEMM_EVENT_POOL.pop(), GEMM_EVENT_POOL.pop()
        e0.record()
        check(lib().ptamd_gemm_group(arr, len(jobs), stream()), "gemm_group")
        e1.record()
        GEMM_TIMING.append((flops, e0, e1, 3, "ptamd_gemm_group dW (staging kernel on a group + one split-K reduce, NPROD=3)"))
        GEMM_BYTES.append(nbytes)


def colsum(x, out, accumulate=True):
    T, N = x.shape
    ws = workspace("colsum", lib().ptamd_colsum_workspace_bytes(N), x.device)
    check(lib().ptamd_colsum(ptr(x), T, N, x.stride(0), int(accumulate), ptr(out), ptr(ws), ws.numel(), stream()),
          "colsum")
    return out


def layernorm_fwd(x, gamma, beta, row_scale=None, planes=None):
    T, D = x.shape
    if isinstance(x, PendingRows):
        r = x.residual
        x.value, y = torch.empty_like(r), torch.empty_like(r)
        mean = torch.empty(T, dtype=torch.float32, device=r.device)
        rstd = torch.empty(T, dtype=torch.float32, device=r.device)
# ... 57 lines not shown
        check(lib().ptamd_layernorm_bwd_reduce(arr, len(chunk), stream()), "layernorm_bwd_reduce")
    del pending[:]


def layernorm_bwd_dropout(dy, x, gamma, mean, rstd, dgamma, dbeta, dres, dropout_p, seed, stream_id, row_scale=None,
                          bound_factor=None, bound_scale=None, row_scale_min=None, bound_scale_min=None, pending=None,
                          planes=None):
    T, D = x.shape
    dx = torch.empty_like(x)
    dropped = torch.empty_like(x) if dropout_p > 0 else None
    if pending is not None and len(pending) >= 16:
        layernorm_bwd_flush(pending)
    ws = _ln_workspace(D, x.device, pending)
    defer = pending is not None
    slabs, slab_stride = (dy.n, dy.stride) if isinstance(dy, Slabs) else (1, 0)
    check(lib().ptamd_layernorm_bwd_dropout(ptr(dy), ptr(x), ptr(gamma), ptr(mean), ptr(rstd), ptr(dres), T, D, float(dropout_p),
                                            int(seed), int(stream_id), ptr(dx), ptr(dropped), ptr(row_scale),
                                            ptr(bound_factor), ptr(bound_scale), ptr(row_scale_min), ptr(bound_scale_min),
                                            ptr(planes), None if defer else ptr(dgamma), None if defer else ptr(dbeta),
                                            slabs, slab_stride, ptr(ws), ws.numel(),
                                            stream()), "layernorm_bwd_dropout")
    if defer:
        pending.append((ws, D, dgamma, dbeta))
    return dx, (dropped if dropped is not None else dx)


def weight_scales(jobs):
    from ._lib import WScaleJob
    for i in range(0, len(jobs), 40):
        chunk = jobs[i:i + 40]
        arr = (WScaleJob * len(chunk))()
        for k, j in enumerate(chunk):
            w = j["w"]
            rows, cols = (w.shape[0], w.shape[1]) if w.dim() == 2 else (1, w.shape[0])
            arr[k] = WScaleJob(w=w.data_ptr(), rows=rows, cols=cols, ld=w.stride(0) if w.dim() == 2 else cols,
                               row_scale=j["row_scale"].data_ptr() if j.get("row_scale") is not None else None,
                               col_scale=j["col_scale"].data_ptr() if j.get("col_scale") is not None else None,
                               stats=j["stats"].data_ptr() if j.get("stats") is not None else None,
                               rows_only=int(bool(j.get("rows_only", False))))
        check(lib().ptamd_weight_scales(arr, len(chunk), stream()), "weight_scales")


def bound_scales(jobs):
    from ._lib import BoundJob
    P = lambda t: t.data_ptr() if t is not None else None
    for i in range(0, len(jobs), 40):
        chunk = jobs[i:i + 40]
        arr = (BoundJob * len(chunk))()
        for k, j in enumerate(chunk):
            arr[k] = BoundJob(ln_gamma_stats=P(j.get("ln_gamma")), ln_beta_stats=P(j.get("ln_beta")), w_stats=P(j["w"]),
                              w_stat_index=int(j["w_index"]), bias_stats=P(j.get("bias")), sqrt_d=float(j.get("sqrt_d", 0.0)),
                              post_scale=float(j.get("post_scale", 1.0)), out_scale=P(j.get("out_scale")),
                              out_value=P(j.get("out_value")))
        check(lib().ptamd_bound_scales(arr, len(chunk), stream()), "bound_scales")


def layernorm_bwd(dy, x, gamma, mean, rstd, dgamma, dbeta, dres=None, pending=None):
    T, D = x.shape
    dx = torch.empty_like(x)
    if pending is not None and len(pending) >= 16:
        layernorm_bwd_flush(pending)
    ws = _ln_workspace(D, x.device, pending)
    defer = pending is not None
    check(lib().ptamd_layernorm_bwd(ptr(dy), ptr(x), ptr(gamma), ptr(mean), ptr(rstd), ptr(dres), T, D, ptr(dx),
                                    None if defer else ptr(dgamma), None if defer else ptr(dbeta), ptr(ws), ws.numel(), stream()),
          "layernorm_bwd")
# ... 165 lines not shown


class WeightsPrep:

    def __init__(self, numel, segs, groups, ints, values, nstats):
        import numpy as np
        from ._lib import WprepBound, WprepPlan, WprepSeg
        dev = ints.device
        RB, PF = lib().ptamd_wprep_rows_per_block(), lib().ptamd_wprep_plain_floats_per_block()
        PANEL = 512
        segs = sorted(segs, key=lambda s: s["offset"])
        idx = lambda view, base: -1 if view is None else view.storage_offset() - base.storage_offset()
        table, blocks_a, blocks_b, plain = [], [], [], []
        ncolmax = ncolsq = 0
        pos = 0
        for s in segs:
            rows, cols, off = int(s["rows"]), int(s["cols"]), int(s["offset"])
            if cols % 4 or off % 4 or off < pos or (cols > PANEL and cols % PANEL):
                raise ValueError(f"ptamd_weights_prep: segment (offset {off}, {rows} x {cols}) is not representable")
            if off > pos:
                plain.append((pos, off - pos))
            pos = off + rows * cols
            want_cols = s.get("col_scale") is not None
            for name in ("row_planes", "col_planes"):
                if s.get(name) is not None and (rows % 32 or cols % 32):
                    raise ValueError("ptamd_weights_prep: planes need rows and cols that are multiples of 32")
            if s.get("col_planes") is not None and not want_cols:
                raise ValueError("ptamd_weights_prep: col_planes need col_scale")
            if s.get("colnorm") and (s.get("stats") is None or not want_cols):
                raise ValueError("ptamd_weights_prep: colnorm needs a statistics record and col_scale")
            stats = -1 if s.get("stats") is None else int(s["stats"])
            npanels = -(-cols // PANEL)
            wide = npanels > 1
            if wide and (s.get("row_planes") is not None or int(s.get("stats_row0", 0)) != 0):
                raise ValueError("ptamd_weights_prep: a matrix wider than 512 columns cannot have row planes or a statistics sub-range")
            colmax0 = ncolmax
            ncolmax += cols if want_cols else 0
            rowmax0 = -1
            if wide and s.get("row_scale") is not None:
                rowmax0 = ncolmax
                ncolmax += rows
            nrb = -(-rows // RB)
            for pnl in range(npanels):
                pc = min(PANEL, cols - pnl * PANEL)
                k = len(table)
                table.append(WprepSeg(
                    offset=off + pnl * PANEL, rows=rows, cols=pc, stats_row0=-1 if wide else int(s.get("stats_row0", 0)),
                    stats_index=stats, row_scale_index=-1 if wide else idx(s.get("row_scale"), ints),
                    col_scale_index=idx(s.get("col_scale"), ints) + pnl * PANEL if want_cols else -1,
                    colmax_index=colmax0 + pnl * PANEL if want_cols else 0,
                    colsq_index=ncolsq if s.get("colnorm") else -1,
                    row_planes=0 if s.get("row_planes") is None else s["row_planes"].data_ptr(), col_planes=0,
                    ld=cols, rowmax_index=rowmax0))
                blocks_a += [(k, b) for b in range(nrb)]
                if want_cols:
                    blocks_b.append((0, k, 0, 0))
                if s.get("colnorm"):
                    ncolsq += nrb * pc
            if wide and rowmax0 >= 0 or s.get("col_planes") is not None:
                k = len(table)
                table.append(WprepSeg(offset=off, rows=rows, cols=cols, stats_row0=0, stats_index=-1,
                                      row_scale_index=idx(s.get("row_scale"), ints) if wide else -1, col_scale_index=-1,
                                      colmax_index=colmax0, colsq_index=-1, row_planes=0,
                                      col_planes=0 if s.get("col_planes") is None else s["col_planes"].data_ptr(), ld=cols,
                                      rowmax_index=rowmax0))
                if rowmax0 >= 0:
                    blocks_b += [(3, k, b, 0) for b in range(-(-rows // 256))]
                if s.get("col_planes") is not None:
                    nchunks = (cols // 32) * (-(-rows // 32) * 2) * 64
                    blocks_b += [(1, k, b, 0) for b in range(-(-nchunks // 256))]
        if pos < numel:
            plain.append((pos, numel - pos))
        arr = (WprepSeg * len(table))(*table)
        n_matrix_blocks = len(blocks_a)
        for j, (first, n) in enumerate(plain):
            blocks_a += [(-(j + 1), b) for b in range(-(-n // PF))]
        by_stats = {}
        for k, t in enumerate(table):
            if t.colsq_index >= 0:
                by_stats.setdefault(int(t.stats_index), []).append(k)
        bounds, grp_rows, cn_list = [], [], []
        rec = lambda v: -1 if v is None else int(v)
        for g, jobs in enumerate(groups):
            first, cn_first = len(bounds), len(cn_list)
            for j in jobs:
                bounds.append(WprepBound(ln_gamma_stats=rec(j.get("ln_gamma")), ln_beta_stats=rec(j.get("ln_beta")), w_stats=int(j["w"]),
                                         w_stat_index=int(j["w_index"]), bias_stats=rec(j.get("bias")),
                                         sqrt_d=float(j.get("sqrt_d", 0.0)), post_scale=float(j.get("post_scale", 1.0)),
                                         out_scale=idx(j.get("out_scale"), ints), out_value=idx(j.get("out_value"), values)))
                if int(j["w_index"]) == 1 and int(j["w"]) in by_stats:
                    cn_list += [k for k in by_stats[int(j["w"])] if k not in cn_list[cn_first:]]
            grp_rows.append((first, len(bounds) - first, cn_first, len(cn_list) - cn_first))
            blocks_b.append((2, g, 0, 0))
        if not groups:
            raise ValueError("ptamd_weights_prep: at least one bounds group (it also resets the statistics)")
        up = lambda a, dt: torch.from_numpy(np.ascontiguousarray(np.asarray(a, dtype=dt))).to(dev)
        self.t_segs = torch.frombuffer(bytearray(bytes(arr)), dtype=torch.uint8).to(dev)
        self.t_blocks_a = up(blocks_a, np.int32).reshape(-1, 2)
        self.t_plain = up(plain if plain else [(0, 0)], np.int64).reshape(-1, 2)
        self.t_blocks_b = up(blocks_b, np.int32).reshape(-1, 4)
# ... 44 lines not shown
```

protein_transformer_amd/models/encoder_only.py:

```python
import collections
import math

import numpy as np
import torch
import torch.nn as nn

from .. import kernels as K
from ..protein.Structure import NUM_PREDICTED_ANGLES

_SITE_ATTN, _SITE_ATTN_OUT, _SITE_FFN_HID, _SITE_FFN_OUT = 0, 1, 2, 3


class _Holder(nn.Module):

    def __init__(self, **shapes):
        super().__init__()
        for name, shape in shapes.items():
            self.register_parameter(name, nn.Parameter(torch.empty(*shape)))


class _AttnHolder(nn.Module):
    def __init__(self, dm):
        super().__init__()
        for nm in ("wq", "wk", "wv", "wo"):
# ... 187 lines not shown
                assert k % 2 != 0, "Kernel size must be odd to maintain sequence length."
                dout = dmodel if (i == len(ks) - 1 and conv_out_matches_dm) else int(din // dr)
                self.conv_shapes.append((din, dout, k))
                din = dout
            if conv_out_matches_dm:
                self.dlayer = dmodel
            else:
                d = dmodel if self.use_embedding else len(vocab)
                for dr in drs:
                    d /= dr
                self.dlayer = int(d)
        D = self.dlayer
        assert D % nhead == 0, "The dimension of the model must be evenly divisible by the number of attn heads."
        widths = [dmodel, D, dff] + [c for _, c, _ in (self.conv_shapes or [])]
        if any(w % 4 for w in widths) or (D // nhead) not in (8, 16, 32, 64, 128):
            raise ValueError("libptamd needs channel widths that are multiples of 4 and width / n_head in {8, 16, 32, 64, 128}")
        self.encoder = _EncoderHolder(len(vocab), dmodel, D, dff, nlayers, max_seq_len, self.conv_shapes,
                                      self.use_embedding)
        self.output_projection = _Holder(weight=(NUM_PREDICTED_ANGLES * 2, D), bias=(NUM_PREDICTED_ANGLES * 2,))
        self._flat = None
        self._flat_grad = None
        self._layout = self._make_layout()
        self.dropout_seed = 0x5DEECE66D
        self._step_counter = 0
        self.grad_hook = None
        self.attn_row_scales = True
        self.attn_mode = None
        self.gemm_mode = None
        self.hp_forward = True
        self.hp_qkv = True
        self.keep_attn_bits = True
        self.ffn_gate_mask = True
        self.hp_dx = True
        self.side_stream_dw = True
        self.top_layer_scales = True
        self.dw_group = "auto"
        self.kv_planes = True
        self.weights_prep = True
        self.auto_guard = AutoGuard(nlayers)
        self._init_parameters()

    def _make_layout(self):
        order = ["encoder.input_embedding.emb.weight"] if self.use_embedding else []
        for j in range(len(self.conv_shapes or [])):
            order += [f"encoder.conv_layers.{j}.weight", f"encoder.conv_layers.{j}.bias"]
        for i in range(self.nlayers):
            b = f"encoder.enc_layers.{i}."
            order += [b + f"self_attn.{n}.weight" for n in ("wq", "wk", "wv")]
            order += [b + f"self_attn.{n}.bias" for n in ("wq", "wk", "wv")]
            order += [b + "self_attn.wo.weight", b + "self_attn.wo.bias",
                      b + "pwff.layer1.weight", b + "pwff.layer1.bias", b + "pwff.layer2.weight", b + "pwff.layer2.bias",
                      b + "sublayer_connections.0.norm.weight", b + "sublayer_connections.0.norm.bias",
                      b + "sublayer_connections.1.norm.weight", b + "sublayer_connections.1.norm.bias"]
        order += ["output_projection.weight", "output_projection.bias"]
        params = dict(self.named_parameters())
        assert set(order) == set(params)
        layout, off = {}, 0
        for name in order:
            shape = tuple(params[name].shape)
            layout[name] = (off, shape)
            off += (int(np.prod(shape)) + 3) // 4 * 4
        self._flat_numel = off
        return layout

    def _init_parameters(self):
        for name, p in self.named_parameters():
# ... 181 lines not shown
                          dict(w=W(b + "pwff.layer1.bias"), stats=st[8])]
                sq = math.sqrt(D)
                bjobs += [dict(ln_gamma=st[3], ln_beta=st[4], w=st[0], w_index=0, bias=st[7], sqrt_d=sq,
                               post_scale=1.0 / (1.0 - pa), out_scale=L["att_scale"]),
                          dict(ln_gamma=st[5], ln_beta=st[6], w=st[1], w_index=0, bias=st[8], sqrt_d=sq,
                               post_scale=1.0 / (1.0 - p), out_scale=L["f1_scale"]),
                          dict(w=st[2], w_index=1, post_scale=1.0 / (1.0 - p), out_value=L["dz1_factor"]),
                          dict(ln_gamma=st[3], ln_beta=st[4], w=ones, w_index=0, sqrt_d=sq, out_scale=L["h1_scale"]),
                          dict(ln_gamma=st[5], ln_beta=st[6], w=ones, w_index=0, sqrt_d=sq, out_scale=L["h2_scale"])]
                layers.append(L)
            assert o == n_i
            dq_stats = torch.zeros(self.nlayers, 4, dtype=torch.float32, device=dev)
            gstats = torch.zeros(self.nlayers, len(AutoGuard.SITES), 4, dtype=torch.float32, device=dev)
            for i, L in enumerate(layers):
                L["dqkv_stats"] = dq_stats[i]
                L["minbuf"] = minbuf
                L["guard_stats"], L["ints"] = gstats, ints
                L["top_stats"] = top_stats
            cache = caches[key] = dict(layers=layers, wjobs=wjobs, bjobs=bjobs,
                                       keep=(ints, stats, factor, ones, dq_stats, minbuf, gstats, top_stats))
            cache["hp_mats"], cache["hp_outs"] = [], []
            cache["hpT_mats"], cache["hpT_scales"], cache["hpT_outs"] = [], [], []
            if D % 32 == 0 and D <= 2048:
                for i, L in enumerate(layers):
                    w1 = W(f"encoder.enc_layers.{i}.pwff.layer1.weight")
                    L["hp_1"] = K.hp_view(torch.empty(K.lib().ptamd_hp_bytes(F, D), dtype=torch.uint8, device=dev), L["rs_1p"], F, D)
                    L["hp_qkv"] = K.hp_view(torch.empty(K.lib().ptamd_hp_bytes(3 * D, D), dtype=torch.uint8, device=dev),
                                            L["rs_qkv"], 3 * D, D)
                    cache["hp_mats"] += [w1, self._qkv(flat, i)[0]]
                    cache["hp_outs"] += [L["hp_1"], L["hp_qkv"]]
                    w2 = W(f"encoder.enc_layers.{i}.pwff.layer2.weight")
                    planes2 = torch.empty(K.lib().ptamd_hp_bytes(F, D), dtype=torch.uint8, device=dev)
                    L["hp_2t"] = K.hp_view(planes2, L["cs_2"], F, D)
                    cache["hpT_mats"] += [w2]
                    cache["hpT_scales"] += [L["cs_2"]]
                    cache["hpT_outs"] += [L["hp_2t"]]
            panels_ok = all(c <= 512 or c % 512 == 0 for c in (D, F))
            cache["prep"] = self._build_prep(cache, p, pa) if (F <= 2048 and D % 4 == 0 and F % 4 == 0 and panels_ok) else None
        need_planes = bool(cache["hp_mats"]) and bool(hp)
        if self.weights_prep and cache.get("prep") is not None:
            stamp = self._weights_stamp()
            fresh = cache.get("fresh")
            if fresh is None or fresh[0] != stamp or (need_planes and not fresh[1]):
                cache["prep"].prepare(self._flat, with_planes=need_planes)
                cache["fresh"] = (stamp, need_planes)
                self.__dict__["_prep_launches"] = self.__dict__.get("_prep_launches", 0) + 1
            if self.training and backward:
                self.__dict__["_train_cache"] = (cache, need_planes)
            return cache["layers"]
        K.weight_scales(cache["wjobs"])
        K.bound_scales(cache["bjobs"])
        if cache["hp_mats"] and hp:
            if self.hp_qkv:
                K.hp_split_rows(cache["hp_mats"], cache["hp_outs"])
            else:
                K.hp_split_rows(cache["hp_mats"][0::2], cache["hp_outs"][0::2])
            if self.hp_dx and F % 32 == 0 and backward:
                K.hp_split_cols(cache["hpT_mats"], cache["hpT_scales"], cache["hpT_outs"])
        return cache["layers"]

    def _build_prep(self, cache, p, pa):
        D, F = self.dlayer, self.dff
        layers = cache["layers"]
        ints, factor = cache["keep"][0], cache["keep"][2]
        off = lambda name: self._layout[name][0]
        planes_ok = bool(cache["hp_mats"])
        segs, groups = [], []
        for i, L in enumerate(layers):
            b = f"encoder.enc_layers.{i}."
            r = lambda k, i=i: 9 * i + k
            segs += [
                dict(offset=off(b + "self_attn.wq.weight"), rows=3 * D, cols=D, row_scale=L["rs_qkv"], col_scale=L["cs_qkv"],
                     stats=r(0), stats_row0=2 * D, row_planes=L["hp_qkv"].planes if planes_ok else None),
                dict(offset=off(b + "self_attn.wq.bias") + 2 * D, rows=1, cols=D, stats=r(7)),
                dict(offset=off(b + "self_attn.wo.weight"), rows=D, cols=D, row_scale=L["rs_o"], col_scale=L["cs_o"]),
                dict(offset=off(b + "pwff.layer1.weight"), rows=F, cols=D, row_scale=L["rs_1"], col_scale=L["cs_1"], stats=r(1),
                     row_planes=L["hp_1"].planes if planes_ok else None),
                dict(offset=off(b + "pwff.layer1.bias"), rows=1, cols=F, stats=r(8)),
                dict(offset=off(b + "pwff.layer2.weight"), rows=D, cols=F, row_scale=L["rs_2"], col_scale=L["cs_2"], stats=r(2),
                     colnorm=True, col_planes=L["hp_2t"].planes if (planes_ok and F % 32 == 0) else None),
                dict(offset=off(b + "sublayer_connections.0.norm.weight"), rows=1, cols=D, stats=r(3)),
                dict(offset=off(b + "sublayer_connections.0.norm.bias"), rows=1, cols=D, stats=r(4)),
                dict(offset=off(b + "sublayer_connections.1.norm.weight"), rows=1, cols=D, stats=r(5)),
                dict(offset=off(b + "sublayer_connections.1.norm.bias"), rows=1, cols=D, stats=r(6))]
            sq = math.sqrt(D)
            groups.append([
                dict(ln_gamma=r(3), ln_beta=r(4), w=r(0), w_index=0, bias=r(7), sqrt_d=sq, post_scale=1.0 / (1.0 - pa),
                     out_scale=L["att_scale"]),
                dict(ln_gamma=r(5), ln_beta=r(6), w=r(1), w_index=0, bias=r(8), sqrt_d=sq, post_scale=1.0 / (1.0 - p),
                     out_scale=L["f1_scale"]),
                dict(w=r(2), w_index=1, post_scale=1.0 / (1.0 - p), out_value=L["dz1_factor"]),
                dict(ln_gamma=r(3), ln_beta=r(4), w=-1, w_index=0, sqrt_d=sq, out_scale=L["h1_scale"]),
                dict(ln_gamma=r(5), ln_beta=r(6), w=-1, w_index=0, sqrt_d=sq, out_scale=L["h2_scale"])])
        return K.WeightsPrep(self._flat_numel, segs, groups, ints, factor.view(-1), 9 * self.nlayers)

    def _slice(self, buf, name):
        cache = self.__dict__.setdefault("_view_cache", {})
        ptr = buf.data_ptr()
        key = (ptr, name)
        v = cache.get(key)
        if v is None:
            off, shape = self._layout[name]
            v = buf[off:off + int(np.prod(shape))].view(shape)
            if (self._flat is not None and ptr == self._flat.data_ptr()) or \
                    (self._flat_grad is not None and ptr == self._flat_grad.data_ptr()):
                cache[key] = v.detach()
                v = cache[key]
        return v

    def _qkv(self, buf, i):
        cache = self.__dict__.setdefault("_view_cache", {})
        key = (buf.data_ptr(), "qkv", i)
        v = cache.get(key)
# ... 29 lines not shown
        self.attn_dropout = float(p if attn_p is None else attn_p)


class _PassPlan:
    def __init__(self, m, seq, seed, backward):
        (B, L), D = seq.shape, m.dlayer
        self.B, self.L, self.D, self.H, self.backward, self.seed = B, L, D, m.nhead, backward, seed
        self.p, self.pa = (m.dropout, m.attn_dropout) if m.training else (0.0, 0.0)
        self.arith = ar = K.get_gemm_mode() if m.gemm_mode is None else int(m.gemm_mode)
        self.attn_arith = ar if m.attn_mode is None else int(m.attn_mode)
        if ar == K.GEMM_AUTO and B * L * D < AUTO_F16X2_MIN_WORK:
            self.arith = K.GEMM_BF16X3
        self.fuse = D <= 1024
        self.side = None
        if backward and m.side_stream_dw and D >= 512 and B * L >= SIDE_STREAM_MIN_TOKENS and B * L * D <= SIDE_STREAM_MAX_WORK:
            if m.__dict__.get("_side_stream") is None or m._side_stream.device != seq.device:
                m.__dict__["_side_stream"] = torch.cuda.Stream(device=seq.device)
            self.side = m._side_stream
        self.dw_group = m.dw_group
        if self.dw_group == "auto":
            ffn_tiles = -(-D // 256) * -(-m.dff // 128) + -(-m.dff // 256) * -(-D // 128)
            self.dw_group = "pairs" if ffn_tiles * B * L >= 256 * 2048 else "layer"

    def take_scales(self, m, flat):
        B, L, D, H, attn = self.B, self.L, self.D, self.H, self.attn_arith
        want_hp = B * L >= HP_MIN_TOKENS and bool(m.hp_forward)
        scales = self.scales = m._step_scales(flat, self.arith, self.p, self.pa, hp=want_hp, backward=self.backward)
        self.use_hp = want_hp and scales is not None and "hp_1" in scales[0]
        self.hp_qkv = self.use_hp and m.hp_qkv
        self.kv_planes = self.hp_qkv and m.kv_planes and K.attention_reads_kv_planes(B, L, H, D // H, attn)
        self.keep_bits = self.pa > 0.0 and m.keep_attn_bits and self.backward and K.attention_bwd_reads_keep_bits(B, L, H, D // H, attn)
        self.gate_mask = m.ffn_gate_mask and self.backward
        self.hp_dx = self.use_hp and m.hp_dx and self.fuse and "hp_2t" in scales[0] and m.dff % 32 == 0
        self.attn_row_scales = scales is not None and m.attn_row_scales and K.attention_row_scales_available(D // H, attn)
        self.top_scales = scales is not None and self.fuse and m.top_layer_scales
        guard = self.guard = m.auto_guard if (scales is not None and m.auto_guard.enabled) else None
        self.measure, self.measure_fwd, self.off, self.wide = False, False, None, None
        if guard is not None:
            guard.poll()
            if m.training and self.backward:
                self.measure = guard.want_measure()
                guard.count_step()
            else:
                self.measure_fwd = guard.want_measure_forward()
                guard.eval_passes += 1
            self.off, self.wide = guard.off.copy(), guard.wide.copy()

    def prod(self, i, k, **scale_kw):
        if self.wide is not None and self.wide[i, k]:
            return dict(arith=K.GEMM_BF16X3)
        return dict(arith=self.arith, **scale_kw)


_Acts = collections.namedtuple("_Acts", "x mean1 rstd1 h1 qkv att lse x2 mean2 rstd2 h2 f1 kbits fmask kv")


def _layer_fwd(plan, m, flat, seq, i, x, hplanes):
    Tn, D, H, p, seed, dev = plan.B * plan.L, plan.D, plan.H, plan.p, plan.seed, x.device
    W = lambda name: m._slice(flat, name)
    b = f"encoder.enc_layers.{i}."
    sid = i * 8
    sc = plan.scales[i] if plan.scales is not None else None
    wqkv, bqkv = m._qkv(flat, i)
    s_h1 = torch.empty(Tn, dtype=torch.int32, device=dev) if sc else None
    hp_q = plan.hp_qkv and not (plan.wide is not None and plan.wide[i, 0])
    h1, mean1, rstd1 = K.layernorm_fwd(x, W(b + "sublayer_connections.0.norm.weight"),
                                       W(b + "sublayer_connections.0.norm.bias"), row_scale=s_h1,
                                       planes=hplanes if hp_q else None)
    if isinstance(x, K.PendingRows):
        x = x.value
    kv = None
    if hp_q and plan.kv_planes:
        kv = K.attention_kv_buffers(Tn, H, dev)
        m.__dict__["_kv_plane_passes"] = m.__dict__.get("_kv_plane_passes", 0) + 1
    if hp_q:
        qkv = K.gemm_hp(K.hp_view(hplanes, s_h1, Tn, D), sc["hp_qkv"],
                        torch.empty(Tn, 3 * D, dtype=torch.float32, device=dev), bias=bqkv, kv=kv, kv_col0=D, kv_heads=H)
    else:
        qkv = K.linear_fwd(h1, wqkv, bqkv, **plan.prod(i, 0, a_scale=s_h1, b_scale=sc and sc["rs_qkv"]))
    kbits = None
    if plan.keep_bits:
        kbits = K.attention_keep_bits(plan.B, plan.L, H, dev)
        m.__dict__["_attn_bits_passes"] = m.__dict__.get("_attn_bits_passes", 0) + 1
    att, lse = K.attention_fwd(qkv, seq, H, plan.pa, seed, sid + _SITE_ATTN, arith=plan.attn_arith, keep_bits=kbits, kv=kv)
    use_b = sc is not None and not (plan.off is not None and plan.off[i, 0])
    x2 = K.linear_fwd(att, W(b + "self_attn.wo.weight"), W(b + "self_attn.wo.bias"), residual=x, ldr=D,
                      dropout_p=p, seed=seed, stream_id=sid + _SITE_ATTN_OUT,
                      **plan.prod(i, 1, a_scale=sc["att_scale"] if use_b else None, a_scale_stride=0 if use_b else 1,
                                  b_scale=sc and sc["rs_o"]))
    s_h2 = torch.empty(Tn, dtype=torch.int32, device=dev) if sc else None
    h2, mean2, rstd2 = K.layernorm_fwd(x2, W(b + "sublayer_connections.1.norm.weight"),
                                       W(b + "sublayer_connections.1.norm.bias"), row_scale=s_h2, planes=hplanes)
    fmask = None
    if plan.use_hp and not (plan.wide is not None and plan.wide[i, 2]):
        if plan.gate_mask:
            fmask = K.gate_mask_buffer(Tn, m.dff, dev)
            m.__dict__["_gate_mask_passes"] = m.__dict__.get("_gate_mask_passes", 0) + 1
        f1 = K.gemm_hp(K.hp_view(hplanes, s_h2, Tn, D), sc["hp_1"],
                       torch.empty(Tn, m.dff, dtype=torch.float32, device=dev), bias=W(b + "pwff.layer1.bias"),
                       flags=K.EPI_RELU, dropout_p=p, seed=seed, stream_id=sid + _SITE_FFN_HID, gate_mask_out=fmask)
    else:
        f1 = K.linear_fwd(h2, W(b + "pwff.layer1.weight"), W(b + "pwff.layer1.bias"), flags=K.EPI_RELU,
                          dropout_p=p, seed=seed, stream_id=sid + _SITE_FFN_HID,
                          **plan.prod(i, 2, a_scale=s_h2, b_scale=sc and sc["rs_1"]))
    use_b = sc is not None and not (plan.off is not None and plan.off[i, 1])
    x3 = K.linear_fwd(f1, W(b + "pwff.layer2.weight"), W(b + "pwff.layer2.bias"), residual=x2, ldr=D,
                      dropout_p=p, seed=seed, stream_id=sid + _SITE_FFN_OUT, defer_reduce=i + 1 < m.nlayers,
                      **plan.prod(i, 3, a_scale=sc["f1_scale"] if use_b else None, a_scale_stride=0 if use_b else 1,
                                  b_scale=sc and sc["rs_2"]))
    if plan.measure_fwd:
        gs = sc["guard_stats"][i]
        K.weight_scales([dict(w=t, stats=gs[j], rows_only=True) for j, t in ((0, att), (1, f1), (3, h1), (4, h2))])
    return x3, _Acts(x, mean1, rstd1, h1, qkv, att, lse, x2, mean2, rstd2, h2, f1, kbits, fmask, kv)


class _GradSchedule:
    def __init__(self, model, plan, main):
        self.model, self.side, self.group, self.main = model, plan.side, plan.dw_group, main
        self.queue = []
        self.ln_pending = []
        self.keep = []

    def run(self, fn, *args, keep=(), **kw):
        if self.side is None:
            return fn(*args, **kw)
        self.side.wait_stream(self.main)
        self.keep.extend(keep)
        with torch.cuda.stream(self.side):
            return fn(*args, **kw)

    def later(self, dy, x, gw, gb, arith=None, dy_scale=None, x_scale=None):
        if self.group == "off":
            return self.run(K.linear_bwd_weight, dy, x, gw, gb, keep=(dy, x), arith=arith, dy_scale=dy_scale, x_scale=x_scale)
        self.queue.append((dy, x, gw, gb, arith, dy_scale, x_scale))

    def flush(self):
        jobs, self.queue = self.queue, []
        ok = [j for j in jobs if j[5] is not None and j[6] is not None and j[1].shape[1] % 4 == 0]
        tiles = sum(-(-j[0].shape[1] // 256) * -(-j[1].shape[1] // 128) for j in ok)
        sk = K.pick_group_split(tiles, ok[0][0].shape[0]) if 2 <= len(ok) <= 4 else 0
        if sk < 2:
            ok = []
# ... 14 lines not shown
        if hook is not None:
            K.layernorm_bwd_flush(self.ln_pending)
            self.run(hook, *self.model._span(first, last))


def _layer_bwd(plan, m, flat, gflat, seq, i, a, carry, dws, s_dqkv_all, dy2_planes):
    dx, dy2, s_dy2, bs_dz1, have_min, have_planes = carry
    D, H, p, pa, seed, ar, fuse, dev = plan.D, plan.H, plan.p, plan.pa, plan.seed, plan.arith, plan.fuse, dx.device
    W = lambda name: m._slice(flat, name)
    G = lambda name: m._slice(gflat, name)
    i32 = lambda: torch.empty(plan.B * plan.L, dtype=torch.int32, device=dev)
    scales, wide = plan.scales, plan.wide
    b = f"encoder.enc_layers.{i}."
    sid = i * 8
    sc = scales[i] if scales is not None else None
    if dy2 is None:
        dy2 = K.dropout_bwd(dx, p, seed, sid + _SITE_FFN_OUT) if p > 0 else dx
        if plan.top_scales:
            ts = sc["top_stats"]
            K.weight_scales([dict(w=dy2, stats=ts, rows_only=True)])
            K.bound_scales([dict(w=ts, w_index=2, out_scale=sc["dy2_min"]),
                            dict(ln_gamma=sc["dz1_factor_rec"], sqrt_d=1.0, w=ts, w_index=0, out_scale=sc["dz1_min"])])
            have_min = True
    uni = sc is not None and have_min
    o_att, o_f1, o_dz1, o_h1, o_h2 = (bool(v) for v in plan.off[i]) if plan.off is not None else (False,) * 5
    dws.later(dy2, a.f1, G(b + "pwff.layer2.weight"), G(b + "pwff.layer2.bias"), arith=ar,
              dy_scale=sc["dy2_min"] if uni and not o_f1 else None, x_scale=sc["f1_scale"] if uni and not o_f1 else None)
    if dy2_planes is not None and have_planes and not (wide is not None and wide[i, 7]):
        dz1 = K.gemm_hp(K.hp_view(dy2_planes, s_dy2, plan.B * plan.L, D), sc["hp_2t"],
                        torch.empty(plan.B * plan.L, m.dff, dtype=torch.float32, device=dev),
                        residual=a.f1 if a.fmask is None else None, ldr=a.f1.stride(0) if a.fmask is None else 0,
                        gate_mask=a.fmask, flags=K.EPI_GATE, gate_scale=1.0 / (1.0 - p))
    else:
        dz1 = K.linear_bwd_input(dy2, W(b + "pwff.layer2.weight"), gate=a.f1, gate_dropout_p=p, gate_mask=a.fmask,
                                 **plan.prod(i, 7, a_scale=s_dy2 if sc else None, b_scale=sc and sc["cs_2"]))
    if plan.measure:
        gs = sc["guard_stats"][i]
        K.weight_scales([dict(w=t, stats=gs[j], rows_only=True) for j, t in enumerate((a.att, a.f1, dz1, a.h1, a.h2))])
    uni1 = uni and not (o_dz1 or o_h2)
    dws.later(dz1, a.h2, G(b + "pwff.layer1.weight"), G(b + "pwff.layer1.bias"), arith=ar,
              dy_scale=sc["dz1_min"] if uni1 else None, x_scale=sc["h2_scale"] if uni1 else None)
    if dws.group != "layer":
        dws.flush()
    dh2 = K.linear_bwd_input(dz1, W(b + "pwff.layer1.weight"), defer_reduce=fuse,
                             **plan.prod(i, 6, a_scale=bs_dz1 if sc and not o_dz1 else None, b_scale=sc and sc["cs_1"]))
    g2w, g2b = G(b + "sublayer_connections.1.norm.weight"), G(b + "sublayer_connections.1.norm.bias")
    if fuse:
        s_dyo = i32() if sc else None
        dx2, dyo = K.layernorm_bwd_dropout(dh2, a.x2, W(b + "sublayer_connections.1.norm.weight"), a.mean2, a.rstd2, g2w, g2b,
                                           dx, p, seed, sid + _SITE_ATTN_OUT, row_scale=s_dyo,
                                           row_scale_min=sc["dyo_min"] if sc else None, pending=dws.ln_pending)
    else:
        s_dyo = None
        dx2 = K.layernorm_bwd(dh2, a.x2, W(b + "sublayer_connections.1.norm.weight"), a.mean2, a.rstd2, g2w, g2b, dres=dx,
                              pending=dws.ln_pending)
        dyo = K.dropout_bwd(dx2, p, seed, sid + _SITE_ATTN_OUT) if p > 0 else dx2
    uni_o = sc is not None and fuse and not o_att
    dws.later(dyo, a.att, G(b + "self_attn.wo.weight"), G(b + "self_attn.wo.bias"), arith=ar,
              dy_scale=sc["dyo_min"] if uni_o else None, x_scale=sc["att_scale"] if uni_o else None)
    datt = K.linear_bwd_input(dyo, W(b + "self_attn.wo.weight"), **plan.prod(i, 5, a_scale=s_dyo, b_scale=sc and sc["cs_o"]))
    s_dqkv = s_dqkv_all[i] if plan.attn_row_scales else None
    dqkv = K.attention_bwd(a.qkv, seq, a.att, datt, a.lse, H, pa, seed, sid + _SITE_ATTN, arith=plan.attn_arith,
                           row_scale=s_dqkv, row_scale_min=sc["dqkv_min"] if plan.attn_row_scales else None, keep_bits=a.kbits,
                           kv=a.kv)
    gw, gb = m._qkv(gflat, i)
    dq_uni = sc["dqkv_min"] if sc is not None else None
    if sc is not None and not plan.attn_row_scales:
# ... 127 lines not shown
```

Baseline: 1.618 million residues/s.

## Store FFN hidden activation as pre-split f16 planes instead of f32

```diff
diff --git a/include/ptamd.h b/include/ptamd.h
--- a/include/ptamd.h
+++ b/include/ptamd.h
@@ -80,6 +80,7 @@
   const uint32_t *a_scale; int a_scale_stride;
   const uint32_t *b_scale; int b_scale_stride;
   const uint64_t *gate_mask;
+  const void *b_planes;
 } ptamd_gemm_args;
 size_t ptamd_gate_mask_bytes(int M, int N);
 size_t ptamd_gemm_workspace_bytes(int M, int N, int split_k);
@@ -118,6 +119,8 @@
   const uint64_t *gate_mask;
   uint64_t *gate_mask_out;
   void *kv_planes; float *kv_inv; int kv_col0, kv_heads;
+  int a_scale_uniform;
+  void *c_planes; const float *c_plane_scale;
 } ptamd_gemm_hp_args;
 size_t ptamd_gemm_hp_workspace_bytes(int M, int N, int split_k);
 int ptamd_gemm_hp(const ptamd_gemm_hp_args *args, void *stream);
@@ -126,6 +129,7 @@
   const float *w; int rows, cols, ld;
   uint32_t *row_scale; uint32_t *col_scale; float *stats;
   int rows_only;
+  const void *planes; const uint32_t *plane_scale;
 } ptamd_wscale_job;
 int ptamd_weight_scales(const ptamd_wscale_job *jobs_host, int njobs, void *stream);
 typedef struct {
diff --git a/protein_transformer_amd/_lib.py b/protein_transformer_amd/_lib.py
--- a/protein_transformer_amd/_lib.py
+++ b/protein_transformer_amd/_lib.py
@@ -32,12 +32,13 @@
                 ("reserved_cus", _i),
                 ("a_scale", _p), ("a_scale_stride", _i),
                 ("b_scale", _p), ("b_scale_stride", _i),
-                ("gate_mask", _p)]
+                ("gate_mask", _p),
+                ("b_planes", _p)]
 
 
 class WScaleJob(C.Structure):
     _fields_ = [("w", _p), ("rows", _i), ("cols", _i), ("ld", _i), ("row_scale", _p), ("col_scale", _p), ("stats", _p),
-                ("rows_only", _i)]
+                ("rows_only", _i), ("planes", _p), ("plane_scale", _p)]
 
 
 class BoundJob(C.Structure):
@@ -71,7 +72,8 @@
                 ("gate_scale", _f),
                 ("reserved_cus", _i),
                 ("gate_mask", _p), ("gate_mask_out", _p),
-                ("kv_planes", _p), ("kv_inv", _p), ("kv_col0", _i), ("kv_heads", _i)]
+                ("kv_planes", _p), ("kv_inv", _p), ("kv_col0", _i), ("kv_heads", _i),
+                ("a_scale_uniform", _i), ("c_planes", _p), ("c_plane_scale", _p)]
 
 
 class WprepSeg(C.Structure):
diff --git a/protein_transformer_amd/csrc/gemm.hip b/protein_transformer_amd/csrc/gemm.hip
--- a/protein_transformer_amd/csrc/gemm.hip
+++ b/protein_transformer_amd/csrc/gemm.hip
@@ -369,11 +369,11 @@
 namespace {
 int build_params(const ptamd_gemm_args *a, GemmParams &p, int &splits, int &mode, float *&user_c) {
   if (!a || a->M <= 0 || a->N <= 0 || a->K <= 0 || !valid_arith(a->arith)) return PTAMD_ERR_BAD_SHAPE;
-  if ((a->lda & 3) || (a->ldb & 3)) return PTAMD_ERR_BAD_SHAPE;
+  if ((a->lda & 3) || (!a->b_planes && (a->ldb & 3))) return PTAMD_ERR_BAD_SHAPE;
   if ((!a->a_kmajor || !a->b_kmajor) && (a->K & 3)) return PTAMD_ERR_BAD_SHAPE;
   if (a->a_kmajor && (a->M & 3)) return PTAMD_ERR_BAD_SHAPE;
   if (a->b_kmajor && (a->N & 3)) return PTAMD_ERR_BAD_SHAPE;
-  if (!pt_aligned16(a->A) || !pt_aligned16(a->B)) return PTAMD_ERR_ALIGN;
+  if (!pt_aligned16(a->A) || !pt_aligned16(a->B) || !pt_aligned16(a->b_planes)) return PTAMD_ERR_ALIGN;
   if (a->dropout_p < 0.f || a->dropout_p >= 1.f) return PTAMD_ERR_BAD_SHAPE;
   splits = a->split_k > 1 ? a->split_k : 1;
   constexpr int BK = 32;
@@ -413,6 +413,15 @@
     if (a->colsum) p.colsum = p.C + (size_t)splits * p.slab;
   }
   mode = resolve_mode(a);
+  p.b_planes = 0;
+  if (a->b_planes) {
+    if (!a->a_kmajor || !a->b_kmajor || mode != PTAMD_GEMM_F16X2 || !a->a_scale || !a->b_scale || a->b_scale_stride != 0 ||
+        (a->K & 31) || (a->N & 7) || splits < 2)
+      return PTAMD_ERR_BAD_SHAPE;
+    p.b_planes = 1;
+    p.B = static_cast<const float *>(a->b_planes);
+    p.ldb = (a->N + 31) / 32 * 32;
+  }
   if (a->gate_mask && (mode != PTAMD_GEMM_F16X2 || !p.vec_epilogue || splits > 1 || a->dropout_p != 0.f)) return PTAMD_ERR_BAD_SHAPE;
   p.scale_a = p.scale_b = nullptr;
   p.scale_a_stride = p.scale_b_stride = 1;
diff --git a/protein_transformer_amd/csrc/gemm_common.h b/protein_transformer_amd/csrc/gemm_common.h
--- a/protein_transformer_amd/csrc/gemm_common.h
+++ b/protein_transformer_amd/csrc/gemm_common.h
@@ -37,6 +37,7 @@
   const uint64_t *gate_mask;
   uint64_t *gate_mask_out;
   int mask_rb, mask_cb;
+  int b_planes;
 };
 __device__ __forceinline__ uint32_t load_gate_masks(const GemmParams &p, int rb, int cb, int lane) {
   const int rbu = __builtin_amdgcn_readfirstlane(rb), cbu = __builtin_amdgcn_readfirstlane(cb);
diff --git a/protein_transformer_amd/csrc/gemm_f16x2.hip b/protein_transformer_amd/csrc/gemm_f16x2.hip
--- a/protein_transformer_amd/csrc/gemm_f16x2.hip
+++ b/protein_transformer_amd/csrc/gemm_f16x2.hip
@@ -121,10 +121,18 @@
   return pt_check_launch();
 }
 
-int launch_group_f16x2(const GemmGroup &g, hipStream_t st) { return launch_group<3>(g, st); }
+int launch_group_f16x2(const GemmGroup &g, hipStream_t st) {
+  for (int j = 0; j < g.n; ++j)
+    if (g.p[j].b_planes) return launch_group<3, true>(g, st);
+  return launch_group<3>(g, st);
+}
 
 int launch_split_f16x2(const GemmParams &p, bool a_kmajor, bool b_kmajor, int splits, hipStream_t st) {
   const bool plain = p.slab != 0 || (!p.bias && !p.residual && !p.flags && p.dropout_p == 0.f);
+  if (p.b_planes) {
+    if (!a_kmajor || !b_kmajor || p.slab == 0) return PTAMD_ERR_BAD_SHAPE;
+    return launch_ti<true, true, 3, EPI_PLAIN, 4, true>(p, splits, st);
+  }
   if (plain) return launch_layout<3, EPI_PLAIN>(p, a_kmajor, b_kmajor, splits, st);
   if (p.dropout_p == 0.f) return launch_layout<3, EPI_NODROP>(p, a_kmajor, b_kmajor, splits, st);
   return launch_layout<3, EPI_FULL>(p, a_kmajor, b_kmajor, splits, st);
diff --git a/protein_transformer_amd/csrc/gemm_hp.hip b/protein_transformer_amd/csrc/gemm_hp.hip
--- a/protein_transformer_amd/csrc/gemm_hp.hip
+++ b/protein_transformer_amd/csrc/gemm_hp.hip
@@ -25,6 +25,10 @@
   char *kv_planes;
   float *kv_inv;
   int kv_col0, kv_heads, kv_nt;
+  int a_scale_stride;
+  char *c_planes;
+  const float *c_plane_scale;
+  int c_kb16;
 };
 
 typedef __attribute__((address_space(1))) const void *gptr_t;
@@ -184,7 +188,7 @@
           for (int g = 0; g < 4; ++g)
 #pragma unroll
             for (int e = 0; e < 4; ++e) {
-              const float ia = inverse_of_scale(p.a_scale[min(row0 + i * 32 + 8 * g + 4 * lh + e, p.g.M - 1)]);
+              const float ia = inverse_of_scale(p.a_scale[min(row0 + i * 32 + 8 * g + 4 * lh + e, p.g.M - 1) * p.a_scale_stride]);
 #pragma unroll
               for (int j = 0; j < 2; ++j) acc[i][j][g * 4 + e] = acc[i][j][g * 4 + e] * ia * ib[j];
             }
@@ -212,7 +216,7 @@
 
 typedef HpGeom<4, 2, 2, true> Geom;
 
-template <int EPI, bool KVP = false>
+template <int EPI, bool KVP = false, bool PLN = false>
 int launch_hp3(const HpParams &p, int splits, hipStream_t st);
 template <int EPI>
 int launch_hp(const HpParams &p, int splits, hipStream_t st) {
@@ -246,7 +250,7 @@
   return v;
 }
 
-template <int EPI, bool KVP = false>
+template <int EPI, bool KVP = false, bool PLN = false>
 __device__ __forceinline__ void hp3_epilogue(const GemmParams &p, const f32x16 (&acc)[2][2], float *C, int ldc, bool partial,
                                              int row0, int col0, int lane, uint32_t thr, float keep_scale, float *scratch,
                                              const HpParams *hp = nullptr) {
@@ -254,6 +258,8 @@
   using ptgemm::EPI_PLAIN;
   typedef float f32x4 __attribute__((ext_vector_type(4)));
   const int l31 = lane & 31, lh = lane >> 5;
+  float plane_scale = 1.f;
+  if (PLN) plane_scale = *hp->c_plane_scale;
   uint32_t keep[2] = {0xffffffffu, 0xffffffffu};
   if (EPI == EPI_FULL && !partial && p.dropout_p > 0.f) {
     keep[0] = keep[1] = 0u;
@@ -341,6 +347,20 @@
         }
         continue;
       }
+      if (PLN) {
+        const int rr = lane >> 3, ch = lane & 7;
+        const float4 a = *reinterpret_cast<const float4 *>(scratch + rr * 64 + ch * 8);
+        const float4 b = *reinterpret_cast<const float4 *>(scratch + rr * 64 + ch * 8 + 4);
+        const int row = row0 + i * 32 + 8 * g + rr, col = col0 + ch * 8;
+        if (row < p.M && col < p.N) {
+          uint4 hi, lo;
+          kv_split8(a, b, plane_scale, hi, lo);
+          char *dst = hp->c_planes + block_offset(row >> 5, col >> 4, 0, hp->c_kb16) + chunk_index(row & 31, (col >> 3) & 1) * 16;
+          *reinterpret_cast<uint4 *>(dst) = hi;
+          *reinterpret_cast<uint4 *>(dst + BLK_BYTES) = lo;
+        }
+        continue;
+      }
 #pragma unroll
       for (int u = 0; u < 2; ++u) {
         const int f = lane + 64 * u, rr = f >> 4, c4 = (f & 15) * 4;
@@ -385,7 +405,7 @@
 
 #define PT_DS_READ_B128(dst, addr, off) asm volatile("ds_read_b128 %0, %1 offset:%2" : "=v"(dst) : "v"(addr), "n"(off))
 
-template <int EPI, bool KVP = false>
+template <int EPI, bool KVP = false, bool PLN = false>
 __global__ __launch_bounds__(Hp3::THREADS, 2) void gemm_hp3_kernel(const HpParams p) {
   using G = Hp3;
   extern __shared__ __attribute__((aligned(16))) char smem[];
@@ -525,12 +545,12 @@
           for (int g = 0; g < 4; ++g)
 #pragma unroll
             for (int e = 0; e < 4; ++e) {
-              const float ia = inverse_of_scale(p.a_scale[min(row0 + i * 32 + 8 * g + 4 * lh + e, p.g.M - 1)]);
+              const float ia = inverse_of_scale(p.a_scale[min(row0 + i * 32 + 8 * g + 4 * lh + e, p.g.M - 1) * p.a_scale_stride]);
 #pragma unroll
               for (int j = 0; j < 2; ++j) acc[i][j][g * 4 + e] = acc[i][j][g * 4 + e] * ia * ib[j];
             }
       }
-      hp3_epilogue<EPI, KVP>(p.g, acc, C, ldc, partial, row0, col0, lane, thr, keep_scale, scratch + wave * 512, &p);
+      hp3_epilogue<EPI, KVP, PLN>(p.g, acc, C, ldc, partial, row0, col0, lane, thr, keep_scale, scratch + wave * 512, &p);
       zero_acc();
     }
     if (!advance(cc)) break;
@@ -538,10 +558,10 @@
   }
 }
 
-template <int EPI, bool KVP>
+template <int EPI, bool KVP, bool PLN>
 int launch_hp3(const HpParams &p, int splits, hipStream_t st) {
   const int work = ((p.g.M + Hp3::TILE_M - 1) / Hp3::TILE_M) * ((p.g.N + HBN - 1) / HBN) * splits;
-  auto kern = gemm_hp3_kernel<EPI, KVP>;
+  auto kern = gemm_hp3_kernel<EPI, KVP, PLN>;
   PT_HIP_TRY(hipFuncSetAttribute(reinterpret_cast<const void *>(kern), hipFuncAttributeMaxDynamicSharedMemorySize, (int)Hp3::LDS));
   const int slots = ptgemm::persistent_grid(p.g.reserved_cus);
   hipLaunchKernelGGL(kern, dim3(work < slots ? work : slots), dim3(Hp3::THREADS), Hp3::LDS, st, p);
@@ -789,7 +809,7 @@
 
 int ptamd_gemm_hp(const ptamd_gemm_hp_args *a, void *stream) {
   if (!a || a->M <= 0 || a->N <= 0 || a->K <= 0) return PTAMD_ERR_BAD_SHAPE;
-  if (!a->A || !a->B || !a->A_scale || !a->B_scale || !a->C) return PTAMD_ERR_BAD_SHAPE;
+  if (!a->A || !a->B || !a->A_scale || !a->B_scale || (!a->C && !a->c_planes)) return PTAMD_ERR_BAD_SHAPE;
   if (!pt_aligned16(a->A) || !pt_aligned16(a->B)) return PTAMD_ERR_ALIGN;
   if (a->dropout_p < 0.f || a->dropout_p >= 1.f) return PTAMD_ERR_BAD_SHAPE;
   if ((a->flags & PTAMD_EPI_GATE) && (a->residual == nullptr) == (a->gate_mask == nullptr)) return PTAMD_ERR_BAD_SHAPE;
@@ -802,7 +822,7 @@
   g.dropout_p = a->dropout_p; g.seed = a->seed; g.stream_id = a->stream_id; g.gate_scale = a->gate_scale;
   g.reserved_cus = a->reserved_cus;
   g.colsum = nullptr; g.colsum_share = 1; g.scale_a = g.scale_b = nullptr; g.scale_a_stride = g.scale_b_stride = 1;
-  g.gate_mask = a->gate_mask; g.gate_mask_out = a->gate_mask_out;
+  g.gate_mask = a->gate_mask; g.gate_mask_out = a->gate_mask_out; g.b_planes = 0;
   g.mask_rb = (a->M + 31) / 32; g.mask_cb = (a->N + 31) / 32;
   constexpr int HBK = 32;
   const int Kp = round_up(a->K, 32), stages = Kp / HBK;
@@ -832,7 +852,19 @@
   p.kv_col0 = a->kv_col0;
   p.kv_heads = a->kv_heads;
   p.kv_nt = a->M / 32;
+  p.a_scale_stride = a->a_scale_uniform ? 0 : 1;
+  p.c_planes = static_cast<char *>(a->c_planes);
+  p.c_plane_scale = a->c_plane_scale;
+  p.c_kb16 = kb16(a->N);
   hipStream_t st = (hipStream_t)stream;
+  if (a->c_planes) {
+    if (!a->c_plane_scale || (a->M & 31) || (a->N & 31) || splits > 1 || a->residual || a->gate_mask || a->kv_planes ||
+        (a->flags & ~PTAMD_EPI_RELU))
+      return PTAMD_ERR_BAD_SHAPE;
+    if (!pt_aligned16(a->c_planes)) return PTAMD_ERR_ALIGN;
+    g.C = nullptr; g.ldc = a->N; g.vec_epilogue = 1;
+    return launch_hp3<ptgemm::EPI_FULL, false, true>(p, 1, st);
+  }
   if (a->kv_planes) {
     if (!a->kv_inv || a->kv_heads <= 0 || (a->M & 31) || (a->kv_col0 & 63) || a->kv_col0 < 0 ||
         a->N != a->kv_col0 + 2 * a->kv_heads * 64 || !g.vec_epilogue || splits > 1 || a->residual || a->gate_mask ||
diff --git a/protein_transformer_amd/csrc/gemm_split_kernel.h b/protein_transformer_amd/csrc/gemm_split_kernel.h
--- a/protein_transformer_amd/csrc/gemm_split_kernel.h
+++ b/protein_transformer_amd/csrc/gemm_split_kernel.h
@@ -133,6 +133,24 @@
 #pragma unroll
   for (int i = 0; i < NV; ++i) store_split_f16_one<G, KMAJOR, ROWS>(s, pt, v[i], sc, i);
 }
+template <typename G, int ROWS>
+__device__ __forceinline__ void plane_offsets(int rows, int r0, int pt, uint32_t (&voff)[G::template nv<ROWS>()]) {
+  constexpr int NV = G::template nv<ROWS>();
+  static_assert(G::SBK == 32 && NV * NPRODUCER * 16 == ROWS * 32 * 2 * 2, "a stage = one block row of hp planes");
+  const int kb_last = (rows + 31) / 32 * 2 - 1;
+#pragma unroll
+  for (int i = 0; i < NV; ++i) {
+    const int q = pt + NPRODUCER * i;
+    voff[i] = (uint32_t)(min((r0 >> 4) + (q >> 7), kb_last) * 2 + ((q >> 6) & 1)) * 1024u + (uint32_t)(q & 63) * 16u;
+  }
+}
+template <typename G, int ROWS>
+__device__ __forceinline__ void store_planes_one(unsigned short *__restrict__ s, int pt, const float4 &v, int i) {
+  constexpr int PLANE = G::template plane<ROWS>(), LD_KR = ROWS + KR_PAD;
+  const int q = pt + NPRODUCER * i, c = q & 63, r = c >> 1, h = (c & 1) ^ ((r >> 3) & 1);
+  const int off = ((q >> 6) & 1) * PLANE + r * LD_KR + (q >> 7) * 16 + h * 8;
+  *reinterpret_cast<float4 *>(s + off) = v;
+}
 __device__ __forceinline__ uint32_t row_scale_bits(uint32_t amax) { return min(268u - (amax >> 23), 254u) << 23; }
 __device__ __forceinline__ float inverse_scale(uint32_t scale_bits) { return __uint_as_float((254u << 23) - scale_bits); }
 
@@ -169,7 +187,7 @@
 struct KernelArg<true> {
   typedef GemmGroup type;
 };
-template <bool A_KMAJOR, bool B_KMAJOR, int NPROD, int EPI, int TI = 4, bool GROUPED = false>
+template <bool A_KMAJOR, bool B_KMAJOR, int NPROD, int EPI, int TI = 4, bool GROUPED = false, bool BPL = false>
 __global__ __launch_bounds__(NTHREADS, 1) __attribute__((amdgpu_waves_per_eu(2, 2))) void gemm_bf16x3_mfma_kernel(
     const typename KernelArg<GROUPED>::type arg) {
   extern __shared__ __attribute__((aligned(16))) unsigned short smem[];
@@ -181,6 +199,7 @@
   float *const cs_area = scratch + SCRATCH_FLOATS;
 
   constexpr bool F16 = NPROD == 3;
+  static_assert(!BPL || (F16 && A_KMAJOR && B_KMAJOR && TI == 4), "pre-split B: the weight-gradient products in f16x2");
   const int tid = threadIdx.x, lane = tid & 63, wave = tid >> 6;
   auto P = [&](int j) __attribute__((always_inline)) -> const GemmParams & {
     if constexpr (GROUPED) return arg.p[j];
@@ -244,8 +263,18 @@
     uint32_t voa[NVA], vob[NVB];
     const float *opA = P(ld.it.pj).A, *opB = P(ld.it.pj).B;
     int op_lda = P(ld.it.pj).lda, op_ldb = P(ld.it.pj).ldb;
+    auto b_offsets = [&]() __attribute__((always_inline)) {
+      if constexpr (BPL) {
+        if (P(ld.it.pj).b_planes) {
+          plane_offsets<G, TBN>(P(ld.it.pj).N, ld.it.bn0, pt, vob);
+          return;
+        }
+      }
+      item_offsets<G, B_KMAJOR, TBN>(op_ldb, P(ld.it.pj).N, ld.it.bn0, pt, vob);
+    };
+    bool st_planes = BPL && P(st.it.pj).b_planes != 0;
     item_offsets<G, A_KMAJOR, TBM>(op_lda, P(ld.it.pj).M, ld.it.bm0, pt, voa);
-    item_offsets<G, B_KMAJOR, TBN>(op_ldb, P(ld.it.pj).N, ld.it.bn0, pt, vob);
+    b_offsets();
     float4 ra[NSETS][NVA], rb[NSETS][NVB];
     float rsa[NSETS][MAX_NV], rsb[NSETS][MAX_NV];
     uint32_t soa[MAX_NV], sob[MAX_NV];
@@ -267,7 +296,7 @@
           op_lda = P(ld.it.pj).lda; op_ldb = P(ld.it.pj).ldb;
         }
         item_offsets<G, A_KMAJOR, TBM>(op_lda, P(ld.it.pj).M, ld.it.bm0, pt, voa);
-        item_offsets<G, B_KMAJOR, TBN>(op_ldb, P(ld.it.pj).N, ld.it.bn0, pt, vob);
+        b_offsets();
         if (F16) {
           scale_offsets<G, A_KMAJOR, TBM>(P(ld.it.pj).M, ld.it.bm0, pt, soa, P(ld.it.pj).scale_a_stride);
           scale_offsets<G, B_KMAJOR, TBN>(P(ld.it.pj).N, ld.it.bn0, pt, sob, P(ld.it.pj).scale_b_stride);
@@ -314,7 +343,14 @@
 #pragma unroll
         for (int i0 = 0; i0 < NVB; i0 += GRP) {
 #pragma unroll
-          for (int i = i0; i < i0 + GRP && i < NVB; ++i) store_split_f16_one<G, B_KMAJOR, TBN>(sb, pt, b[i], sb_, i);
+          for (int i = i0; i < i0 + GRP && i < NVB; ++i) {
+            if constexpr (BPL) {
+              if (st_planes) store_planes_one<G, TBN>(sb, pt, b[i], i);
+              else store_split_f16_one<G, B_KMAJOR, TBN>(sb, pt, b[i], sb_, i);
+            } else {
+              store_split_f16_one<G, B_KMAJOR, TBN>(sb, pt, b[i], sb_, i);
+            }
+          }
           __builtin_amdgcn_sched_barrier(0);
 #pragma unroll
           for (int i = i0; i < i0 + GRP && i < NVB; ++i)
@@ -337,7 +373,10 @@
         const int w_before = st.w;
         const bool was_end = st.end;
         advance(st);
-        if (st.w != w_before) colsum_weights(st.it);
+        if (st.w != w_before) {
+          colsum_weights(st.it);
+          if (BPL) st_planes = P(st.it.pj).b_planes != 0;
+        }
         if (st.end && !was_end) {
 #pragma unroll
           for (int i = 0; i < NVA; ++i) cs_w[i] = 0.f;
@@ -469,11 +508,11 @@
 
 constexpr int TI1_COST_X10 = 4;
 constexpr int TI2_COST_NUM = 3, TI2_COST_DEN = 5;
-template <bool AK, bool BKM, int NPROD, int EPI, int TI>
+template <bool AK, bool BKM, int NPROD, int EPI, int TI, bool BPL = false>
 int launch_ti(const GemmParams &p, int splits, hipStream_t st) {
   using G = Geo<NPROD, TI>;
   const int work = ((p.M + G::TBM - 1) / G::TBM) * ((p.N + TBN - 1) / TBN) * splits;
-  auto kern = gemm_bf16x3_mfma_kernel<AK, BKM, NPROD, EPI, TI>;
+  auto kern = gemm_bf16x3_mfma_kernel<AK, BKM, NPROD, EPI, TI, false, BPL>;
   PT_HIP_TRY(hipFuncSetAttribute(reinterpret_cast<const void *>(kern), hipFuncAttributeMaxDynamicSharedMemorySize,
                                  (int)G::LDS_BYTES));
   const int slots = persistent_grid(p.reserved_cus);
@@ -500,10 +539,10 @@
   return launch_ti<AK, BKM, NPROD, EPI, 4>(p, splits, st);
 }
 
-template <int NPROD>
+template <int NPROD, bool BPL = false>
 int launch_group(const GemmGroup &g, hipStream_t st) {
   using G = Geo<NPROD, 4>;
-  auto kern = gemm_bf16x3_mfma_kernel<true, true, NPROD, EPI_PLAIN, 4, true>;
+  auto kern = gemm_bf16x3_mfma_kernel<true, true, NPROD, EPI_PLAIN, 4, true, BPL>;
   PT_HIP_TRY(hipFuncSetAttribute(reinterpret_cast<const void *>(kern), hipFuncAttributeMaxDynamicSharedMemorySize,
                                  (int)G::LDS_BYTES));
   const int slots = persistent_grid(g.p[0].reserved_cus), work = g.first[g.n];
diff --git a/protein_transformer_amd/csrc/scales.hip b/protein_transformer_amd/csrc/scales.hip
--- a/protein_transformer_amd/csrc/scales.hip
+++ b/protein_transformer_amd/csrc/scales.hip
@@ -1,4 +1,5 @@
 #include "common.h"
+#include "hp_format.h"
 
 namespace {
 
@@ -35,7 +36,21 @@
       if (r >= jb.rows) break;
       const float *p = jb.w + (size_t)r * jb.ld;
       float m = 0.f, sq = 0.f;
-      if (vec) {
+      if (jb.planes) {
+        typedef _Float16 h4 __attribute__((ext_vector_type(4)));
+        const float inv = pthp::inverse_of_scale(__uint_as_float(*jb.plane_scale));
+        const int kbv = pthp::kb16(jb.cols);
+        for (int c = lane * 4; c < jb.cols; c += 256) {
+          const char *src = static_cast<const char *>(jb.planes) + pthp::block_offset(r >> 5, c >> 4, 0, kbv) +
+                            pthp::chunk_index(r & 31, (c >> 3) & 1) * 16 + ((c >> 2) & 1) * 8;
+          const h4 hi = *reinterpret_cast<const h4 *>(src), lo = *reinterpret_cast<const h4 *>(src + pthp::BLK_BYTES);
+          float4 v;
+          v.x = ((float)hi[0] + (float)lo[0]) * inv; v.y = ((float)hi[1] + (float)lo[1]) * inv;
+          v.z = ((float)hi[2] + (float)lo[2]) * inv; v.w = ((float)hi[3] + (float)lo[3]) * inv;
+          m = fmaxf(fmaxf(m, fmaxf(fabsf(v.x), fabsf(v.y))), fmaxf(fabsf(v.z), fabsf(v.w)));
+          sq = fmaf(v.x, v.x, fmaf(v.y, v.y, fmaf(v.z, v.z, fmaf(v.w, v.w, sq))));
+        }
+      } else if (vec) {
         for (int c = lane * 4; c < jb.cols; c += 256) {
           const float4 v = *reinterpret_cast<const float4 *>(p + c);
           m = fmaxf(fmaxf(m, fmaxf(fabsf(v.x), fabsf(v.y))), fmaxf(fabsf(v.z), fabsf(v.w)));
@@ -182,7 +197,11 @@
   int blocks = 0;
   for (int j = 0; j < njobs; ++j) {
     const ptamd_wscale_job &q = jobs[j];
-    if (!q.w || q.rows <= 0 || q.cols <= 0 || q.ld < q.cols) return PTAMD_ERR_BAD_SHAPE;
+    if (q.planes) {
+      if (!q.plane_scale || !q.rows_only || q.col_scale || q.rows <= 0 || q.cols <= 0 || (q.cols & 3)) return PTAMD_ERR_BAD_SHAPE;
+    } else if (!q.w || q.rows <= 0 || q.cols <= 0 || q.ld < q.cols) {
+      return PTAMD_ERR_BAD_SHAPE;
+    }
     js.job[j] = q;
     js.first_block[j] = blocks;
     js.row_blocks[j] = (q.row_scale || q.stats) ? (q.rows + ROWS_PER_BLOCK - 1) / ROWS_PER_BLOCK : 0;
diff --git a/protein_transformer_amd/csrc/wprep.hip b/protein_transformer_amd/csrc/wprep.hip
--- a/protein_transformer_amd/csrc/wprep.hip
+++ b/protein_transformer_amd/csrc/wprep.hip
@@ -289,6 +289,32 @@
     ptsplit::split_pair_f16(v[4], v[5], sc, sc, hi.z, lo.z);
     ptsplit::split_pair_f16(v[6], v[7], sc, sc, hi.w, lo.w);
     char *dst = reinterpret_cast<char *>(sg.col_planes) + pthp::block_offset(rb, kb, 0, kbv) + c * 16;
+    *reinterpret_cast<uint4 *>(dst) = hi;
+    *reinterpret_cast<uint4 *>(dst + pthp::BLK_BYTES) = lo;
+    return;
+  }
+  if (blk.x == 4) {
+    if (!pl.with_planes) return;
+    const ptamd_wprep_seg sg = pl.segs[blk.y];
+    const int kbv = pthp::kb16(sg.cols);
+    const int64_t nchunks = (int64_t)(sg.rows / 32) * kbv * 64;
+    const int64_t id = (int64_t)blk.z * 256 + tid;
+    if (id >= nchunks) return;
+    const int c = (int)(id & 63);
+    const int64_t b = id >> 6;
+    const int kb = (int)(b % kbv), rb = (int)(b / kbv);
+    int r, h;
+    pthp::chunk_coords(c, r, h);
+    const int row = rb * 32 + r, k0 = kb * 16 + h * 8;
+    const float sc = __uint_as_float(pt_row_scale_bits(pl.colmax[sg.rowmax_index + row]));
+    const float *x = w + sg.offset + (size_t)row * sg.ld + k0;
+    const float4 a = *reinterpret_cast<const float4 *>(x), q = *reinterpret_cast<const float4 *>(x + 4);
+    uint4 hi, lo;
+    ptsplit::split_pair_f16(a.x, a.y, sc, sc, hi.x, lo.x);
+    ptsplit::split_pair_f16(a.z, a.w, sc, sc, hi.y, lo.y);
+    ptsplit::split_pair_f16(q.x, q.y, sc, sc, hi.z, lo.z);
+    ptsplit::split_pair_f16(q.z, q.w, sc, sc, hi.w, lo.w);
+    char *dst = reinterpret_cast<char *>(sg.row_planes) + pthp::block_offset(rb, kb, 0, kbv) + c * 16;
     *reinterpret_cast<uint4 *>(dst) = hi;
     *reinterpret_cast<uint4 *>(dst + pthp::BLK_BYTES) = lo;
     return;
diff --git a/protein_transformer_amd/kernels.py b/protein_transformer_amd/kernels.py
--- a/protein_transformer_amd/kernels.py
+++ b/protein_transformer_amd/kernels.py
@@ -16,10 +16,11 @@
 
 def gemm(A, B, C_out, *, M, N, K, lda, ldb, ldc, a_kmajor=False, b_kmajor=False, bias=None, residual=None,
          ldr=0, flags=0, dropout_p=0.0, seed=0, stream_id=0, split_k=1, colsum=None, gate_scale=0.0, arith=None,
-         a_scale=None, a_scale_stride=1, b_scale=None, b_scale_stride=1, gate_mask=None, ws=None):
+         a_scale=None, a_scale_stride=1, b_scale=None, b_scale_stride=1, gate_mask=None, ws=None, b_planes=None):
     if ws is None:
         ws = workspace("gemm", lib().ptamd_gemm_workspace_bytes(M, N, split_k), A.device)
-    args = GemmArgs(M=M, N=N, K=K, A=A.data_ptr(), lda=lda, a_kmajor=int(a_kmajor), B=B.data_ptr(), ldb=ldb,
+    args = GemmArgs(M=M, N=N, K=K, A=A.data_ptr(), lda=lda, a_kmajor=int(a_kmajor), B=B.data_ptr() if B is not None else None, ldb=ldb,
+                    b_planes=b_planes.data_ptr() if b_planes is not None else None,
                     b_kmajor=int(b_kmajor), C=C_out.data_ptr() if C_out is not None else ws.data_ptr(), ldc=ldc,
                     bias=bias.data_ptr() if bias is not None else None,
                     residual=residual.data_ptr() if residual is not None else None, ldr=ldr, flags=flags,
@@ -83,6 +84,31 @@
         self.scale = torch.empty(lib().ptamd_hp_padded_rows(self.rows), dtype=torch.float32, device=device)
 
 
+class ActPlanes:
+    __slots__ = ("planes", "scale", "rows", "K")
+
+    def __init__(self, rows, K, scale, device):
+        self.rows, self.K, self.scale = int(rows), int(K), scale
+        self.planes = torch.empty(lib().ptamd_hp_bytes(self.rows, self.K), dtype=torch.uint8, device=device)
+
+    @property
+    def shape(self):
+        return (self.rows, self.K)
+
+    def to_float(self):
+        kb = -(-self.K // 32) * 2
+        v = self.planes.view(torch.float16).view(-1, kb, 2, 32, 2, 8).float()
+        v = v[:, :, 0] + v[:, :, 1]
+        r = torch.arange(32, device=v.device)
+        flip = ((r >> 3) & 1).bool()
+        v = torch.where(flip[None, None, :, None, None], v.flip(3), v)
+        x = v.permute(0, 2, 1, 3, 4).reshape(-1, kb * 16)[:self.rows, :self.K]
+        return (x / self.scale.view(torch.float32)[0]).contiguous()
+
+    def view(self, *shape):
+        return self.to_float().view(*shape)
+
+
 def hp_split(x, transposed=False, out=None):
     assert x.dim() == 2 and x.stride(1) == 1
     rows, K = (x.shape[1], x.shape[0]) if transposed else (x.shape[0], x.shape[1])
@@ -94,12 +120,19 @@
 
 
 def gemm_hp(a, b, C_out, *, bias=None, residual=None, ldr=0, flags=0, dropout_p=0.0, seed=0, stream_id=0, split_k=1,
-            gate_scale=0.0, gate_mask=None, gate_mask_out=None, kv=None, kv_col0=0, kv_heads=0):
+            gate_scale=0.0, gate_mask=None, gate_mask_out=None, kv=None, kv_col0=0, kv_heads=0, a_uniform=False,
+            c_planes=None):
     assert a.K == b.K
     M, N = a.rows, b.rows
-    ws = workspace("gemm_hp", lib().ptamd_gemm_hp_workspace_bytes(M, N, split_k), C_out.device) if split_k > 1 else None
+    assert (C_out is None) == (c_planes is not None)
+    if c_planes is not None:
+        assert c_planes.shape == (M, N)
+    ws = workspace("gemm_hp", lib().ptamd_gemm_hp_workspace_bytes(M, N, split_k), a.planes.device) if split_k > 1 else None
     args = GemmHpArgs(M=M, N=N, K=a.K, A=a.planes.data_ptr(), A_scale=a.scale.data_ptr(), B=b.planes.data_ptr(),
-                      B_scale=b.scale.data_ptr(), C=C_out.data_ptr(), ldc=C_out.stride(0),
+                      B_scale=b.scale.data_ptr(), C=C_out.data_ptr() if C_out is not None else None,
+                      ldc=C_out.stride(0) if C_out is not None else N, a_scale_uniform=int(bool(a_uniform)),
+                      c_planes=c_planes.planes.data_ptr() if c_planes is not None else None,
+                      c_plane_scale=c_planes.scale.data_ptr() if c_planes is not None else None,
                       bias=bias.data_ptr() if bias is not None else None,
                       residual=residual.data_ptr() if residual is not None else None, ldr=ldr, flags=flags,
                       dropout_p=float(dropout_p), seed=int(seed) & (2 ** 64 - 1), stream_id=int(stream_id),
@@ -119,7 +152,7 @@
         e1.record()
         GEMM_TIMING.append((2.0 * M * N * a.K, e0, e1, 3, "ptamd_gemm_hp (LDS-DMA kernel gemm_hp3_kernel, NPROD=3)"))
         GEMM_BYTES.append(4 * (M * a.K + N * a.K + M * N * (1 + (residual is not None) + bool(flags & EPI_ACCUM))))
-    return C_out
+    return C_out if c_planes is None else c_planes
 
 
 DW_SLOTS = 512
@@ -245,6 +278,12 @@
 def linear_bwd_weight(dy, x, dw, dbias=None, arith=None, dy_scale=None, x_scale=None):
     T, N = dy.shape
     K = x.shape[1]
+    if isinstance(x, ActPlanes):
+        if dy_scale is None or x_scale is None:
+            raise ValueError("linear_bwd_weight: an ActPlanes operand needs the uniform scales of both operands")
+        return gemm(dy, None, dw, M=N, N=K, K=T, lda=dy.stride(0), ldb=K, ldc=dw.stride(0), a_kmajor=True,
+                    b_kmajor=True, flags=EPI_ACCUM, split_k=pick_split_k(N, K, T), colsum=dbias, arith=GEMM_F16X2,
+                    a_scale=dy_scale, a_scale_stride=0, b_scale=x_scale, b_scale_stride=0, b_planes=x.planes)
     if dy_scale is not None and x_scale is not None:
         return gemm(dy, x, dw, M=N, N=K, K=T, lda=dy.stride(0), ldb=x.stride(0), ldc=dw.stride(0), a_kmajor=True,
                     b_kmajor=True, flags=EPI_ACCUM, split_k=pick_split_k(N, K, T), colsum=dbias, arith=GEMM_F16X2,
@@ -274,7 +313,9 @@
         T, N = dy.shape
         Kd = x.shape[1]
         ws = workspace(f"gemm_group{j}", lib().ptamd_gemm_workspace_bytes(N, Kd, split_k), dw.device)
-        arr[j] = GemmArgs(M=N, N=Kd, K=T, A=dy.data_ptr(), lda=dy.stride(0), a_kmajor=1, B=x.data_ptr(), ldb=x.stride(0),
+        pl = isinstance(x, ActPlanes)
+        arr[j] = GemmArgs(M=N, N=Kd, K=T, A=dy.data_ptr(), lda=dy.stride(0), a_kmajor=1, B=None if pl else x.data_ptr(),
+                          ldb=Kd if pl else x.stride(0), b_planes=x.planes.data_ptr() if pl else None,
                           b_kmajor=1, C=dw.data_ptr(), ldc=dw.stride(0), bias=None, residual=None, ldr=0, flags=EPI_ACCUM,
                           dropout_p=0.0, seed=0, stream_id=0, split_k=int(split_k), workspace=ws.data_ptr(),
                           workspace_bytes=ws.numel(), colsum=dbias.data_ptr() if dbias is not None else None, gate_scale=0.0,
@@ -398,6 +439,12 @@
         arr = (WScaleJob * len(chunk))()
         for k, j in enumerate(chunk):
             w = j["w"]
+            if isinstance(w, ActPlanes):
+                arr[k] = WScaleJob(w=None, rows=w.rows, cols=w.K, ld=w.K, row_scale=j["row_scale"].data_ptr() if j.get("row_scale") is not None else None,
+                                   col_scale=None, stats=j["stats"].data_ptr() if j.get("stats") is not None else None,
+                                   rows_only=int(bool(j.get("rows_only", False))), planes=w.planes.data_ptr(),
+                                   plane_scale=w.scale.data_ptr())
+                continue
             rows, cols = (w.shape[0], w.shape[1]) if w.dim() == 2 else (1, w.shape[0])
             arr[k] = WScaleJob(w=w.data_ptr(), rows=rows, cols=cols, ld=w.stride(0) if w.dim() == 2 else cols,
                                row_scale=j["row_scale"].data_ptr() if j.get("row_scale") is not None else None,
@@ -629,8 +676,10 @@
             stats = -1 if s.get("stats") is None else int(s["stats"])
             npanels = -(-cols // PANEL)
             wide = npanels > 1
-            if wide and (s.get("row_planes") is not None or int(s.get("stats_row0", 0)) != 0):
-                raise ValueError("ptamd_weights_prep: a matrix wider than 512 columns cannot have row planes or a statistics sub-range")
+            if wide and int(s.get("stats_row0", 0)) != 0:
+                raise ValueError("ptamd_weights_prep: a matrix wider than 512 columns cannot have a statistics sub-range")
+            if wide and s.get("row_planes") is not None and s.get("row_scale") is None:
+                raise ValueError("ptamd_weights_prep: row_planes of a matrix wider than 512 columns need row_scale")
             colmax0 = ncolmax
             ncolmax += cols if want_cols else 0
             rowmax0 = -1
@@ -647,7 +696,7 @@
                     col_scale_index=idx(s.get("col_scale"), ints) + pnl * PANEL if want_cols else -1,
                     colmax_index=colmax0 + pnl * PANEL if want_cols else 0,
                     colsq_index=ncolsq if s.get("colnorm") else -1,
-                    row_planes=0 if s.get("row_planes") is None else s["row_planes"].data_ptr(), col_planes=0,
+                    row_planes=0 if (wide or s.get("row_planes") is None) else s["row_planes"].data_ptr(), col_planes=0,
                     ld=cols, rowmax_index=rowmax0))
                 blocks_a += [(k, b) for b in range(nrb)]
                 if want_cols:
@@ -658,11 +707,14 @@
                 k = len(table)
                 table.append(WprepSeg(offset=off, rows=rows, cols=cols, stats_row0=0, stats_index=-1,
                                       row_scale_index=idx(s.get("row_scale"), ints) if wide else -1, col_scale_index=-1,
-                                      colmax_index=colmax0, colsq_index=-1, row_planes=0,
+                                      colmax_index=colmax0, colsq_index=-1,
+                                      row_planes=0 if (not wide or s.get("row_planes") is None) else s["row_planes"].data_ptr(),
                                       col_planes=0 if s.get("col_planes") is None else s["col_planes"].data_ptr(), ld=cols,
                                       rowmax_index=rowmax0))
                 if rowmax0 >= 0:
                     blocks_b += [(3, k, b, 0) for b in range(-(-rows // 256))]
+                if wide and s.get("row_planes") is not None:
+                    blocks_b += [(4, k, b, 0) for b in range(-(-((rows // 32) * (cols // 16) * 64) // 256))]
                 if s.get("col_planes") is not None:
                     nchunks = (cols // 32) * (-(-rows // 32) * 2) * 64
                     blocks_b += [(1, k, b, 0) for b in range(-(-nchunks // 256))]
diff --git a/protein_transformer_amd/models/encoder_only.py b/protein_transformer_amd/models/encoder_only.py
--- a/protein_transformer_amd/models/encoder_only.py
+++ b/protein_transformer_amd/models/encoder_only.py
@@ -243,6 +243,7 @@
         self.keep_attn_bits = True
         self.ffn_gate_mask = True
         self.hp_dx = True
+        self.act_planes = True
         self.side_stream_dw = True
         self.top_layer_scales = True
         self.dw_group = "auto"
@@ -490,6 +491,10 @@
                     w2 = W(f"encoder.enc_layers.{i}.pwff.layer2.weight")
                     planes2 = torch.empty(K.lib().ptamd_hp_bytes(F, D), dtype=torch.uint8, device=dev)
                     L["hp_2t"] = K.hp_view(planes2, L["cs_2"], F, D)
+                    if F <= 2048:
+                        L["hp_2"] = K.hp_view(torch.empty(K.lib().ptamd_hp_bytes(D, F), dtype=torch.uint8, device=dev), L["rs_2"], D, F)
+                        cache.setdefault("hp2_mats", []).append(w2)
+                        cache.setdefault("hp2_outs", []).append(L["hp_2"])
                     cache["hpT_mats"] += [w2]
                     cache["hpT_scales"] += [L["cs_2"]]
                     cache["hpT_outs"] += [L["hp_2t"]]
@@ -515,6 +520,8 @@
                 K.hp_split_rows(cache["hp_mats"][0::2], cache["hp_outs"][0::2])
             if self.hp_dx and F % 32 == 0 and backward:
                 K.hp_split_cols(cache["hpT_mats"], cache["hpT_scales"], cache["hpT_outs"])
+            if self.act_planes and F % 32 == 0 and backward and cache.get("hp2_mats"):
+                K.hp_split_rows(cache["hp2_mats"], cache["hp2_outs"])
         return cache["layers"]
 
     def _build_prep(self, cache, p, pa):
@@ -536,7 +543,8 @@
                      row_planes=L["hp_1"].planes if planes_ok else None),
                 dict(offset=off(b + "pwff.layer1.bias"), rows=1, cols=F, stats=r(8)),
                 dict(offset=off(b + "pwff.layer2.weight"), rows=D, cols=F, row_scale=L["rs_2"], col_scale=L["cs_2"], stats=r(2),
-                     colnorm=True, col_planes=L["hp_2t"].planes if (planes_ok and F % 32 == 0) else None),
+                     colnorm=True, col_planes=L["hp_2t"].planes if (planes_ok and F % 32 == 0) else None,
+                     row_planes=L["hp_2"].planes if (planes_ok and F % 32 == 0 and "hp_2" in L) else None),
                 dict(offset=off(b + "sublayer_connections.0.norm.weight"), rows=1, cols=D, stats=r(3)),
                 dict(offset=off(b + "sublayer_connections.0.norm.bias"), rows=1, cols=D, stats=r(4)),
                 dict(offset=off(b + "sublayer_connections.1.norm.weight"), rows=1, cols=D, stats=r(5)),
@@ -632,6 +640,10 @@
         self.keep_bits = self.pa > 0.0 and m.keep_attn_bits and self.backward and K.attention_bwd_reads_keep_bits(B, L, H, D // H, attn)
         self.gate_mask = m.ffn_gate_mask and self.backward
         self.hp_dx = self.use_hp and m.hp_dx and self.fuse and "hp_2t" in scales[0] and m.dff % 32 == 0
+        self.f1_planes = bool(self.use_hp and m.act_planes and self.gate_mask and self.fuse and "hp_2" in scales[0] and
+                              m.dff % 32 == 0 and (B * L) % 32 == 0 and B * L * m.dff * 4 < 2 ** 32 and
+                              K.pick_split_k_rows(B * L, D, m.dff) == 1)
+        self.nlayers = m.nlayers
         self.attn_row_scales = scales is not None and m.attn_row_scales and K.attention_row_scales_available(D // H, attn)
         self.top_scales = scales is not None and self.fuse and m.top_layer_scales
         guard = self.guard = m.auto_guard if (scales is not None and m.auto_guard.enabled) else None
@@ -645,6 +657,13 @@
                 self.measure_fwd = guard.want_measure_forward()
                 guard.eval_passes += 1
             self.off, self.wide = guard.off.copy(), guard.wide.copy()
+
+    def f1_as_planes(self, i):
+        if not self.f1_planes or (self.off is not None and self.off[i, 1]):
+            return False
+        if self.wide is not None and (self.wide[i, 2] or self.wide[i, 3] or self.wide[i, 7]):
+            return False
+        return i + 1 < self.nlayers or bool(self.top_scales)
 
     def prod(self, i, k, **scale_kw):
         if self.wide is not None and self.wide[i, k]:
@@ -696,18 +715,26 @@
         if plan.gate_mask:
             fmask = K.gate_mask_buffer(Tn, m.dff, dev)
             m.__dict__["_gate_mask_passes"] = m.__dict__.get("_gate_mask_passes", 0) + 1
+        f1_pl = plan.f1_as_planes(i)
         f1 = K.gemm_hp(K.hp_view(hplanes, s_h2, Tn, D), sc["hp_1"],
-                       torch.empty(Tn, m.dff, dtype=torch.float32, device=dev), bias=W(b + "pwff.layer1.bias"),
-                       flags=K.EPI_RELU, dropout_p=p, seed=seed, stream_id=sid + _SITE_FFN_HID, gate_mask_out=fmask)
+                       None if f1_pl else torch.empty(Tn, m.dff, dtype=torch.float32, device=dev), bias=W(b + "pwff.layer1.bias"),
+                       flags=K.EPI_RELU, dropout_p=p, seed=seed, stream_id=sid + _SITE_FFN_HID, gate_mask_out=fmask,
+                       c_planes=K.ActPlanes(Tn, m.dff, sc["f1_scale"], dev) if f1_pl else None)
+        if f1_pl:
+            m.__dict__["_act_plane_passes"] = m.__dict__.get("_act_plane_passes", 0) + 1
     else:
         f1 = K.linear_fwd(h2, W(b + "pwff.layer1.weight"), W(b + "pwff.layer1.bias"), flags=K.EPI_RELU,
                           dropout_p=p, seed=seed, stream_id=sid + _SITE_FFN_HID,
                           **plan.prod(i, 2, a_scale=s_h2, b_scale=sc and sc["rs_1"]))
     use_b = sc is not None and not (plan.off is not None and plan.off[i, 1])
-    x3 = K.linear_fwd(f1, W(b + "pwff.layer2.weight"), W(b + "pwff.layer2.bias"), residual=x2, ldr=D,
-                      dropout_p=p, seed=seed, stream_id=sid + _SITE_FFN_OUT, defer_reduce=i + 1 < m.nlayers,
-                      **plan.prod(i, 3, a_scale=sc["f1_scale"] if use_b else None, a_scale_stride=0 if use_b else 1,
-                                  b_scale=sc and sc["rs_2"]))
+    if isinstance(f1, K.ActPlanes):
+        x3 = K.gemm_hp(f1, sc["hp_2"], torch.empty(Tn, D, dtype=torch.float32, device=dev), bias=W(b + "pwff.layer2.bias"),
+                       residual=x2, ldr=D, dropout_p=p, seed=seed, stream_id=sid + _SITE_FFN_OUT, a_uniform=True)
+    else:
+        x3 = K.linear_fwd(f1, W(b + "pwff.layer2.weight"), W(b + "pwff.layer2.bias"), residual=x2, ldr=D,
+                          dropout_p=p, seed=seed, stream_id=sid + _SITE_FFN_OUT, defer_reduce=i + 1 < m.nlayers,
+                          **plan.prod(i, 3, a_scale=sc["f1_scale"] if use_b else None, a_scale_stride=0 if use_b else 1,
+                                      b_scale=sc and sc["rs_2"]))
     if plan.measure_fwd:
         gs = sc["guard_stats"][i]
         K.weight_scales([dict(w=t, stats=gs[j], rows_only=True) for j, t in ((0, att), (1, f1), (3, h1), (4, h2))])
@@ -788,7 +815,8 @@
                         residual=a.f1 if a.fmask is None else None, ldr=a.f1.stride(0) if a.fmask is None else 0,
                         gate_mask=a.fmask, flags=K.EPI_GATE, gate_scale=1.0 / (1.0 - p))
     else:
-        dz1 = K.linear_bwd_input(dy2, W(b + "pwff.layer2.weight"), gate=a.f1, gate_dropout_p=p, gate_mask=a.fmask,
+        dz1 = K.linear_bwd_input(dy2, W(b + "pwff.layer2.weight"), gate=None if isinstance(a.f1, K.ActPlanes) else a.f1,
+                                 gate_dropout_p=p, gate_mask=a.fmask,
                                  **plan.prod(i, 7, a_scale=s_dy2 if sc else None, b_scale=sc and sc["cs_2"]))
     if plan.measure:
         gs = sc["guard_stats"][i]
```

Measured after the change: 1.626 million residues/s (median of 6 runs). Within noise of the previous version (+0.5%).
